# koadman/libMems

Hardware: AMD Instinct MI355X
Metric: seed-mers/sec sorted+matched (+ MUMs/sec) at 1/2/4/8 MI355X; HBM GB/s vs roofline (higher is better)
Workload: dtype u64; 1 GPU; BASELINE config 3: 8 x 100 Mbp, seed weight 19 (0x7b974ef), MemHash seed stage (sorted+matched); genomes=8, genome_length=100000000, seedmers_total=799999792, seedmers_rank0=799999792, probes_rank0=100459493, parallelism=1 GPU

## Files before the change

### libmems_amd/csrc/groups.hip

```cpp
#include <cstdlib>
#include <type_traits>

#include "match_device.h"
#include "seed_device.h"

namespace mums {

namespace {

constexpr int kGTile = kSegTile;
constexpr int kGRounds = kGTile / kBlock;
constexpr int kSlots = kGTile / 2;
#ifndef MUMS_GROUP_SPLIT
#define MUMS_GROUP_SPLIT 2
#endif
constexpr int kGSplit = MUMS_GROUP_SPLIT;
constexpr int kGSub = kGTile / kGSplit;
constexpr int kGSubRounds = kGSub / kBlock;
constexpr int kSubSlots = kGSub / 2;
static_assert(kGSub % kBlock == 0 && kGSubRounds * (kBlock / 64) <= 64, "probe sub-tile");

__device__ __forceinline__ uint32_t blk_excl_scan(uint32_t v, uint32_t* s_w, uint32_t* total) {
    const int lane = threadIdx.x & 63, wv = threadIdx.x >> 6;
    uint32_t inc = v;
// ... 88 lines not shown
    }
    if (nrep) atomicAdd(&ctr->repeat_limit, (unsigned long long)nrep);
    __syncthreads();

    uint32_t base = 0;
    const uint64_t sb = (uint64_t)blockIdx.x * kSlots;
    for (uint32_t c = 0; c < H; c += kBlock) {
        const uint32_t j = c + threadIdx.x;
        const uint32_t vv = j < H ? okb[j] : 0u;
        const uint32_t ok = vv >> 31;
        uint32_t tot;
        const uint32_t o = blk_excl_scan(ok, s_w, &tot);
        if (ok) {
            slot_info[sb + base + o] = (tile0 + heads[j]) | ((uint64_t)gsz16[j] << 32);
            slot_bucket[sb + base + o] = vv & 0x7FFFFFFFu;
        }
        base += tot;
    }
    if (threadIdx.x == 0) {
        tile_count[blockIdx.x] = base;
        tile_count[gridDim.x + 32 + blockIdx.x] = H;
    }
}

typedef __attribute__((address_space(3))) const uint64_t lds_u64;

template <int IB>
struct TileRecViewT {
    lds_u64* lds;
    const uint64_t* glob;
    uint64_t t0;
    uint32_t count;
    __device__ __forceinline__ uint64_t raw(uint64_t i) const {
        const uint64_t k = i - t0;
        return k < count ? lds[k] : glob[i];
    }
    __device__ __forceinline__ uint64_t gkey(uint64_t i) const { return raw(i) >> (IB + 1); }
    __device__ __forceinline__ uint32_t par(uint64_t i) const { return (uint32_t)(raw(i) >> IB) & 1u; }
    __device__ __forceinline__ uint64_t gidx(uint64_t i) const { return raw(i) & ((1ull << IB) - 1); }
    __device__ __forceinline__ RecFields get(uint64_t i) const {
        const uint64_t r = raw(i);
        return RecFields{r >> (IB + 1), (uint32_t)(r >> IB) & 1u, r & ((1ull << IB) - 1)};
    }
};

template <int MG, int IB, bool kGl = false, bool kFastOnly = false>
__global__ __launch_bounds__(kBlock) __attribute__((amdgpu_waves_per_eu(kGl ? 6 : 1))) void probe_tile_rec_kernel(const uint64_t* __restrict__ rec,
                                                                const SegTile* __restrict__ tiles, GenomeTable gt,
                                                                MatchParams mp, int L,
                                                                uint32_t* __restrict__ tile_count,
                                                                uint64_t* __restrict__ slot_info,
                                                                uint32_t* __restrict__ slot_bucket,
                                                                DevCounters* __restrict__ ctr,
                                                                double inv_table) {
    constexpr int kGRounds = kGSubRounds;
    constexpr int kWaves = kBlock / 64;
    __shared__ uint64_t srec[kGSub];
    __shared__ uint16_t heads[kSubSlots];
    __shared__ uint32_t wcnt[kGRounds * kWaves];
    __shared__ uint32_t s_w[2][kWaves];
    __shared__ uint32_t s_ng[kWaves];
    __shared__ uint32_t s_red[2];
    __shared__ uint64_t s_prev, s_next;
    __shared__ uint8_t s_gl[256];
    __shared__ uint32_t s_gb[kMaxG + 1];
    const int lane = threadIdx.x & 63;
    const int wv = __builtin_amdgcn_readfirstlane(threadIdx.x >> 6);
    const SegTile td = tiles[blockIdx.x / kGSplit];
    const uint32_t part0 = (blockIdx.x % kGSplit) * (uint32_t)kGSub;
    if (td.count <= part0) {
        if (threadIdx.x == 0) {
            tile_count[blockIdx.x] = 0;
            tile_count[gridDim.x + 32 + blockIdx.x] = 0;
        }
        return;
    }
    const uint64_t tile0 = td.start + part0;
    const uint32_t cnt = td.count - part0 < (uint32_t)kGSub ? td.count - part0 : (uint32_t)kGSub;

    uint32_t kx[kGRounds];
    {
        uint64_t x[kGRounds];
        #pragma unroll
        for (int r = 0; r < kGRounds; ++r) {
            const uint32_t q = r * kBlock + threadIdx.x;
            x[r] = rec[tile0 + (q < cnt ? q : cnt - 1)];
        }
        #pragma unroll
        for (int r = 0; r < kGRounds; ++r) {
            const uint32_t q = r * kBlock + threadIdx.x;
            if (q < cnt) srec[q] = x[r];
            kx[r] = (uint32_t)(x[r] >> (IB + 1));
        }
    }
    if (threadIdx.x == 0) s_prev = (tile0 > td.bstart) ? rec[tile0 - 1] : ~0ull;
    if (threadIdx.x == 64) s_next = (tile0 + cnt < td.bend) ? rec[tile0 + cnt] : ~0ull;
    constexpr bool use_gl = kGl && IB == 32;
    if constexpr (use_gl) {
        static_assert(kBlock >= 256 && kBlock > kMaxG, "one lookup entry per thread");
        if (threadIdx.x < gt.gl_n) s_gl[threadIdx.x] = gt.gl[threadIdx.x];
        if (threadIdx.x <= kMaxG) s_gb[threadIdx.x] = (uint32_t)gt.base[threadIdx.x];
    }
    const GLook glk{(lds_u8c*)s_gl, (lds_u32c*)s_gb, gt.gl_shift, gt.gl_n ? gt.gl_n - 1 : 0};
    __syncthreads();

    const bool first = tile0 == td.bstart;
    const uint32_t kprev = (uint32_t)(s_prev >> (IB + 1)), knext = (uint32_t)(s_next >> (IB + 1));
// ... 1 lines not shown
    #pragma unroll
    for (int r = 0; r < kGRounds; ++r) ke[r] = 0;
    if (lane == 0 || lane == 63) {
        #pragma unroll
        for (int r = 0; r < kGRounds; ++r) {
            const uint32_t q = r * kBlock + threadIdx.x;
            const uint32_t qe = lane == 0 ? q - 1 : q + 1;
            ke[r] = qe < cnt ? (uint32_t)(srec[qe] >> (IB + 1)) : (lane == 0 ? kprev : knext);
        }
    }
    uint32_t hmask = 0, ngrp = 0;
    #pragma unroll
    for (int r = 0; r < kGRounds; ++r) {
        const uint32_t q = r * kBlock + threadIdx.x;
        const uint32_t here = kx[r];
        const uint32_t prev = (uint32_t)__builtin_amdgcn_update_dpp((int)ke[r], (int)here, 0x138, 0xf, 0xf, false);
        uint32_t next = (uint32_t)__builtin_amdgcn_update_dpp((int)ke[r], (int)here, 0x130, 0xf, 0xf, false);
        next = (q + 1 < cnt) ? next : knext;
        const bool head = q < cnt && ((q == 0 && first) || here != prev);
        const bool keep = head && next == here;
        ngrp += (uint32_t)__popcll(__ballot(head));
        hmask |= (keep ? 1u : 0u) << r;
        const uint64_t bal = __ballot(keep);
        if (lane == 0) wcnt[r * kWaves + wv] = (uint32_t)__popcll(bal);
    }
    if (lane == 0) s_ng[wv] = ngrp;
    __syncthreads();
    if (wv == 0) {
        constexpr int kE = kGRounds * kWaves;
        const uint32_t c0 = lane < kE ? wcnt[lane] : 0u;
        uint32_t inc = c0;
        #pragma unroll
        for (int d = 1; d < 64; d <<= 1) {
            const uint32_t t = __shfl_up(inc, d, 64);
            if (lane >= d) inc += t;
        }
        if (lane < kE) wcnt[lane] = inc - c0;
        if (lane == 63) s_red[0] = inc;
    }
    __syncthreads();
    #pragma unroll
    for (int r = 0; r < kGRounds; ++r) {
        const bool keep = (hmask >> r) & 1u;
        const uint64_t bal = __ballot(keep);
        const uint32_t below = __builtin_amdgcn_mbcnt_hi((uint32_t)(bal >> 32), __builtin_amdgcn_mbcnt_lo((uint32_t)bal, 0u));
        if (keep) heads[wcnt[r * kWaves + wv] + below] = (uint16_t)(r * kBlock + threadIdx.x);
    }
    __syncthreads();
    const uint32_t H = s_red[0];

    const TileRecViewT<IB> v{(lds_u64*)srec, rec, tile0, cnt};
    const bool fast = kFastOnly || (mp.repeat_tol == 0 && mp.enum_tol == 1);
    const uint64_t want_mn = mp.masked ? mp.seq_mask : 0ull;
    const double inv_t = inv_table;
    const uint64_t sb = (uint64_t)blockIdx.x * kSubSlots;
    uint32_t nrep = 0, base = 0, buf = 0;
    for (uint32_t c = 0; c < H; c += kBlock) {
        const uint32_t j = c + threadIdx.x;
        bool ok = false;
        uint32_t gsz = 0, bkt = 0;
        uint64_t h = 0;
        if (j < H) {
            h = tile0 + heads[j];
            int64_t off = 0;
            if (fast) {
                const uint32_t q = heads[j];
                uint64_t xb[MG + 1];
                if (q + (uint32_t)gt.G < cnt) {
                    #pragma unroll
                    for (int k = 0; k <= MG; ++k) {
                        const uint32_t qk = q + ((uint32_t)k <= (uint32_t)gt.G ? (uint32_t)k : 0u);
                        xb[k] = ((uint32_t)k <= (uint32_t)gt.G) ? v.lds[qk] : ~0ull;
                    }
                } else {
                    #pragma unroll
                    for (int k = 0; k <= MG; ++k)
                        xb[k] = ((uint32_t)k <= (uint32_t)gt.G && h + k < td.bend) ? rec[h + k] : ~0ull;
                }
                ok = probe_fast_raw<MG, IB, use_gl>(xb, gt, want_mn, L, &off, &gsz, &glk);
                if (gsz > (uint32_t)gt.G) {
                    uint64_t i = h + gsz;
                    const uint32_t k0 = (uint32_t)(xb[0] >> (IB + 1));
                    while (i < td.bend && gsz <= (uint32_t)kRepeatLimit && (uint32_t)v.gkey(i) == k0) { ++gsz; ++i; }
                }
            } else if constexpr (!kFastOnly) {
                Mhe<MG> P;
                ok = build_probe<MG, TileRecViewT<IB>>(v, h, td.bend, gt, mp, L, P, &gsz);
                off = P.offset;
            }
            nrep += gsz > (uint32_t)kRepeatLimit;
            if (ok) bkt = bucket_of_fast(off, mp.table_size, inv_t);
        }
        const uint64_t bal = __ballot(ok);
        const uint32_t below = __builtin_amdgcn_mbcnt_hi((uint32_t)(bal >> 32), __builtin_amdgcn_mbcnt_lo((uint32_t)bal, 0u));
        if (lane == 0) s_w[buf][wv] = (uint32_t)__popcll(bal);
        __syncthreads();
        uint32_t pre = 0, tot = 0;
        #pragma unroll
        for (int w = 0; w < kWaves; ++w) {
            const uint32_t x = s_w[buf][w];
            pre += (w < wv) ? x : 0u;
            tot += x;
        }
        buf ^= 1u;
        if (ok) {
            const uint32_t o = base + pre + below;
            slot_info[sb + o] = h | ((uint64_t)(gsz > 65535u ? 65535u : gsz) << 32);
            slot_bucket[sb + o] = bkt;
        }
        base += tot;
    }
    if (nrep) atomicAdd(&ctr->repeat_limit, (unsigned long long)nrep);
    if (threadIdx.x == 0) {
        uint32_t gtot = 0;
        #pragma unroll
        for (int w = 0; w < kWaves; ++w) gtot += s_ng[w];
        tile_count[blockIdx.x] = base;
        tile_count[gridDim.x + 32 + blockIdx.x] = gtot;
    }
}

__global__ __launch_bounds__(kBlock) void probe_compact_kernel(const uint32_t* __restrict__ tile_count,
                                                               const uint32_t* __restrict__ tile_off,
                                                               const uint64_t* __restrict__ slot_info,
                                                               const uint32_t* __restrict__ slot_bucket,
                                                               uint64_t* __restrict__ probe_info,
                                                               uint32_t* __restrict__ probe_bucket,
                                                               uint32_t slots_per_block) {
    const uint32_t n = tile_count[blockIdx.x];
    const uint64_t o = tile_off[blockIdx.x];
    const uint64_t sb = (uint64_t)blockIdx.x * slots_per_block;
    for (uint32_t k = threadIdx.x; k < n; k += kBlock) {
        probe_info[o + k] = slot_info[sb + k];
        probe_bucket[o + k] = slot_bucket[sb + k];
    }
}

__global__ void flat_tiles_kernel(uint64_t N, uint64_t nt, SegTile* __restrict__ tiles) {
    const uint64_t t = (uint64_t)blockIdx.x * blockDim.x + threadIdx.x;
    if (t >= nt) return;
    SegTile d{};
    d.start = t * kGTile;
    d.bstart = 0;
    d.bend = N;
    const uint64_t rem = N - d.start;
    d.count = (uint32_t)(rem < (uint64_t)kGTile ? rem : (uint64_t)kGTile);
    d.hbase = 0;
    d.ntb = (uint32_t)nt;
    d.tb = (uint32_t)t;
    tiles[t] = d;
}

#ifndef MUMS_MAT_WIDE
#define MUMS_MAT_WIDE 1
#endif
constexpr bool kMatWide = MUMS_MAT_WIDE != 0;
struct __attribute__((aligned(8))) Rec2 { uint64_t a, b; };

template <int MG, typename View, bool kGl = false>
__global__ __launch_bounds__(kBlock) void probe_materialize_kernel(View v, const uint64_t* __restrict__ probe_info,
                                                                   uint64_t P, GenomeTable gt, MatchParams mp, int L,
                                                                   int64_t* __restrict__ rows, uint64_t* __restrict__ lkey,
                                                                   uint32_t* __restrict__ fsk, uint32_t* __restrict__ lhash,
                                                                   int32_t* __restrict__ rows32) {
    const uint64_t k0 = (uint64_t)blockIdx.x * kBlock;
    const uint64_t k = k0 + threadIdx.x;
    const int W = gt.G + 1;
    Mhe<MG> Q;
    __shared__ uint8_t s_gl[256];
    __shared__ uint32_t s_gb[kMaxG + 1];
    constexpr bool use_gl = kGl && RecIB<View>::value == 32;
    if constexpr (use_gl) {
        for (uint32_t i = threadIdx.x; i < gt.gl_n; i += kBlock) s_gl[i] = gt.gl[i];
        for (int i = threadIdx.x; i <= kMaxG; i += kBlock) s_gb[i] = (uint32_t)gt.base[i];
        __syncthreads();
    }
    const GLook glk{(lds_u8c*)s_gl, (lds_u32c*)s_gb, gt.gl_shift, gt.gl_n ? gt.gl_n - 1 : 0};
    if (k < P) {
        const uint64_t info = probe_info[k];
        const uint64_t h = info & 0xFFFFFFFFull;
        const uint32_t gsz = (uint32_t)((info >> 32) & 0xFFFFull);
        bool done = false;
        if constexpr (RecIB<View>::value > 0) {
            if (mp.repeat_tol == 0 && mp.enum_tol == 1 && gsz <= (uint32_t)MG) {
                uint64_t x[MG];
                if constexpr (MG % 2 == 0 && kMatWide) {
                    #pragma unroll
                    for (int q = 0; q < MG; q += 2) {
                        Rec2 t{~0ull, ~0ull};
                        if ((uint32_t)q < gsz) t = *reinterpret_cast<const Rec2*>(v.rec + h + q);
// ... 13 lines not shown
            build_probe<MG, View>(v, h, h + gsz, gt, mp, L, Q, &gs);
        }
        if (lkey) {
            const uint64_t xs = (uint64_t)start_at(Q, first_start(Q));
            if (lhash) {
                lkey[k] = (xs << 32) | k;
                lhash[k] = line_hash<MG>(Q, gt.G);
            } else {
                lkey[k] = ((uint64_t)line_hash<MG>(Q, gt.G) << 32) | (xs & 0xFFFFFFFFull);
            }
            fsk[k] = (uint32_t)xs;
        }
    }
    if constexpr (MG % 4 == 0 && MG <= 16) {
        if (rows32) {
            if (k >= P) return;
            bool ok = probe_offset<MG>(Q, L) == Q.offset;
            #pragma unroll
            for (int g = 0; g < MG; ++g) ok = ok && Q.s[g] == (int64_t)(int32_t)Q.s[g];
            int32_t* out = rows32 + k * (uint64_t)line_row_stride(gt.G);
            #pragma unroll
            for (int q = 0; q < MG / 4; ++q)
                if (4 * q < gt.G)
                    *reinterpret_cast<int4*>(out + 4 * q) = make_int4((int32_t)Q.s[4 * q], (int32_t)Q.s[4 * q + 1],
                                                                      (int32_t)Q.s[4 * q + 2], (int32_t)Q.s[4 * q + 3]);
            if (!ok) atomicOr(fsk + P, 1u);
            return;
        }
    }
    if constexpr (MG <= 16) {
        __shared__ int64_t srow[kBlock * (MG + 1)];
        if (k < P) {
            int64_t* r = srow + threadIdx.x * W;
            #pragma unroll
            for (int g = 0; g < MG; ++g)
                if (g < gt.G) r[g] = Q.s[g];
            r[gt.G] = Q.offset;
        }
        __syncthreads();
        const uint64_t nk = P - k0 < (uint64_t)kBlock ? P - k0 : (uint64_t)kBlock;
        int64_t* out = rows + k0 * (uint64_t)W;
        for (uint32_t i = threadIdx.x; i < nk * (uint64_t)W; i += kBlock) out[i] = srow[i];
    } else {
        if (k >= P) return;
        int64_t* row = rows + k * (uint64_t)W;
        #pragma unroll
        for (int g = 0; g < MG; ++g)
            if (g < gt.G) row[g] = Q.s[g];
        row[gt.G] = Q.offset;
    }
}

__global__ __launch_bounds__(kBlock) void row_bucket_kernel(const int64_t* __restrict__ rows, uint64_t P, int G,
                                                            uint32_t table_size, double inv_t,
                                                            const uint32_t* __restrict__ bounds, uint32_t nranks,
                                                            uint32_t* __restrict__ out) {
    const uint64_t k = (uint64_t)blockIdx.x * kBlock + threadIdx.x;
    if (k >= P) return;
    const uint32_t b = bucket_of_fast(rows[k * (uint64_t)(G + 1) + G], table_size, inv_t);
    if (!bounds) { out[k] = b; return; }
    uint32_t r = 0;
    while (r + 1 < nranks && bounds[r + 1] <= b) ++r;
    out[k] = r;
}

constexpr int kGatherIPT = 8;
__global__ __launch_bounds__(kBlock) void gather_rows_ilp_kernel(const int64_t* __restrict__ src,
                                                                 const uint32_t* __restrict__ perm, uint64_t n, uint32_t W,
                                                                 int64_t* __restrict__ dst) {
    const uint64_t e0 = (uint64_t)blockIdx.x * (kBlock * kGatherIPT) + threadIdx.x;
    uint64_t k = e0 / W;
    uint32_t c = (uint32_t)(e0 - k * W);
    const uint32_t dk = kBlock / W, dc = kBlock % W;
    int64_t x[kGatherIPT];
    #pragma unroll
    for (int i = 0; i < kGatherIPT; ++i) {
        const uint64_t e = e0 + (uint64_t)i * kBlock;
        x[i] = e < n ? src[(uint64_t)perm[k] * W + c] : 0;
        k += dk;
        c += dc;
        if (c >= W) { c -= W; ++k; }
    }
    #pragma unroll
    for (int i = 0; i < kGatherIPT; ++i) {
        const uint64_t e = e0 + (uint64_t)i * kBlock;
        if (e < n) dst[e] = x[i];
    }
}

__global__ __launch_bounds__(kBlock) void bucket_rec_kernel(const uint32_t* __restrict__ b, uint64_t P,
                                                            uint64_t* __restrict__ rec) {
    const uint64_t k = (uint64_t)blockIdx.x * kBlock + threadIdx.x;
    if (k < P) rec[k] = ((uint64_t)b[k] << 32) | k;
}

__global__ __launch_bounds__(kBlock) void bucket_split_kernel(const uint64_t* __restrict__ rec, uint64_t P,
                                                              uint32_t* __restrict__ b, uint32_t* __restrict__ ids) {
    const uint64_t k = (uint64_t)blockIdx.x * kBlock + threadIdx.x;
    if (k >= P) return;
    const uint64_t r = rec[k];
    b[k] = (uint32_t)(r >> 32);
    ids[k] = (uint32_t)r;
}

__global__ __launch_bounds__(kBlock) void chain_dest_kernel(const uint32_t* __restrict__ fk, uint64_t nch,
                                                            const uint32_t* __restrict__ pdest,
                                                            uint32_t* __restrict__ cdest) {
    const uint64_t c = (uint64_t)blockIdx.x * kBlock + threadIdx.x;
    if (c < nch) cdest[c] = pdest[fk[c]];
}

__global__ __launch_bounds__(kBlock) void inverse_perm_kernel(const uint32_t* __restrict__ perm, uint64_t n,
                                                              uint32_t* __restrict__ inv) {
    const uint64_t k = (uint64_t)blockIdx.x * kBlock + threadIdx.x;
    if (k < n) inv[perm[k]] = (uint32_t)k;
}

__global__ __launch_bounds__(kBlock) void chain_tag_kernel(const uint32_t* __restrict__ chain_of,
                                                           const uint32_t* __restrict__ perm,
                                                           const uint32_t* __restrict__ sdest, uint64_t P,
                                                           const uint32_t* __restrict__ cinv,
                                                           const uint32_t* __restrict__ cstart,
                                                           uint32_t* __restrict__ tags) {
    const uint64_t k = (uint64_t)blockIdx.x * kBlock + threadIdx.x;
    if (k < P) tags[k] = cinv[chain_of[perm[k]]] - cstart[sdest[k]];
}

__global__ __launch_bounds__(kBlock) void chain_entry_out_kernel(const int64_t* __restrict__ pool,
                                                                 const uint32_t* __restrict__ fk,
                                                                 const uint32_t* __restrict__ cperm,
                                                                 const uint32_t* __restrict__ scdest, uint64_t nch,
                                                                 int G, const uint32_t* __restrict__ pinv,
                                                                 const uint32_t* __restrict__ rstart,
                                                                 int64_t* __restrict__ eout, uint32_t* __restrict__ fout) {
    const uint64_t k = (uint64_t)blockIdx.x * kBlock + threadIdx.x;
    if (k >= nch) return;
    const uint32_t c = cperm[k];
    const uint64_t W = (uint64_t)(G + 2);
    for (uint64_t w = 0; w < W; ++w) eout[k * W + w] = pool[(uint64_t)c * W + w];
    if (fout) fout[k] = pinv[fk[c]] - rstart[scdest[k]];
}

__global__ __launch_bounds__(kBlock) void kept_dest_kernel(const int64_t* __restrict__ rows, uint64_t P, int G,
                                                           const uint32_t* __restrict__ chain_of,
                                                           const uint32_t* __restrict__ cinv,
                                                           const uint2* __restrict__ thr,
                                                           const uint32_t* __restrict__ fk,
                                                           const uint32_t* __restrict__ pdest, uint32_t nranks,
                                                           uint32_t* __restrict__ dest) {
    const uint64_t k = (uint64_t)blockIdx.x * kBlock + threadIdx.x;
    if (k >= P) return;
    const uint32_t c = chain_of[k];
    const uint2 t = thr[cinv[c]];
    bool keep = t.y != 0u && fk[c] == (uint32_t)k;
    if (!keep) {
// ... 73 lines not shown

hipError_t launch_inverse_perm(const uint32_t* perm, uint64_t n, uint32_t* inv, hipStream_t st) {
    if (n == 0) return hipSuccess;
    hipLaunchKernelGGL(inverse_perm_kernel, dim3((unsigned)((n + kBlock - 1) / kBlock)), dim3(kBlock), 0, st, perm, n,
                       inv);
    return hipGetLastError();
}

hipError_t launch_chain_tags(const uint32_t* chain_of, const uint32_t* perm, const uint32_t* sdest, uint64_t P,
                             const uint32_t* cinv, const uint32_t* cstart, uint32_t* tags, hipStream_t st) {
    if (P == 0) return hipSuccess;
    hipLaunchKernelGGL(chain_tag_kernel, dim3((unsigned)((P + kBlock - 1) / kBlock)), dim3(kBlock), 0, st, chain_of,
                       perm, sdest, P, cinv, cstart, tags);
    return hipGetLastError();
}

hipError_t launch_chain_entries_out(const int64_t* pool, const uint32_t* fk, const uint32_t* cperm,
                                    const uint32_t* scdest, uint64_t nch, int G, const uint32_t* pinv,
                                    const uint32_t* rstart, int64_t* eout, uint32_t* fout, hipStream_t st) {
    if (nch == 0) return hipSuccess;
    hipLaunchKernelGGL(chain_entry_out_kernel, dim3((unsigned)((nch + kBlock - 1) / kBlock)), dim3(kBlock), 0, st,
                       pool, fk, cperm, scdest, nch, G, pinv, rstart, eout, fout);
    return hipGetLastError();
}

hipError_t launch_kept_dest(const int64_t* rows, uint64_t P, int G, const uint32_t* chain_of, const uint32_t* cinv,
                            const uint2* thr, const uint32_t* fk, const uint32_t* pdest, uint32_t nranks, uint32_t* dest,
                            hipStream_t st) {
    if (P == 0) return hipSuccess;
    hipLaunchKernelGGL(kept_dest_kernel, dim3((unsigned)((P + kBlock - 1) / kBlock)), dim3(kBlock), 0, st, rows, P, G,
                       chain_of, cinv, thr, fk, pdest, nranks, dest);
    return hipGetLastError();
}

hipError_t launch_dest_first(const uint32_t* sdest, uint64_t P, uint32_t* first, hipStream_t st) {
    if (P == 0) return hipSuccess;
    hipLaunchKernelGGL(dest_first_kernel, dim3((unsigned)((P + kBlock - 1) / kBlock)), dim3(kBlock), 0, st, sdest, P,
                       first);
    return hipGetLastError();
}

hipError_t launch_entry_first(const uint32_t* scdest, uint64_t nch, const uint32_t* rcount, const uint32_t* perm,
                              const uint32_t* sdest, uint64_t K, const uint32_t* chain_of, const uint32_t* cinv,
                              const uint32_t* rstart, uint32_t* efirst, hipStream_t st) {
    if (nch == 0) return hipSuccess;
    hipLaunchKernelGGL(entry_first_init_kernel, dim3((unsigned)((nch + kBlock - 1) / kBlock)), dim3(kBlock), 0, st,
                       scdest, nch, rcount, efirst);
    if (K)
        hipLaunchKernelGGL(entry_first_kernel, dim3((unsigned)((K + kBlock - 1) / kBlock)), dim3(kBlock), 0, st, perm,
                           sdest, K, chain_of, cinv, rstart, efirst);
    return hipGetLastError();
}

hipError_t launch_bucket_records(const uint32_t* b, uint64_t P, uint64_t* rec, hipStream_t st) {
    if (P == 0) return hipSuccess;
    hipLaunchKernelGGL(bucket_rec_kernel, dim3((unsigned)((P + kBlock - 1) / kBlock)), dim3(kBlock), 0, st, b, P, rec);
    return hipGetLastError();
}

hipError_t launch_bucket_split(const uint64_t* rec, uint64_t P, uint32_t* b, uint32_t* ids, hipStream_t st) {
    if (P == 0) return hipSuccess;
    hipLaunchKernelGGL(bucket_split_kernel, dim3((unsigned)((P + kBlock - 1) / kBlock)), dim3(kBlock), 0, st, rec, P, b,
                       ids);
    return hipGetLastError();
}

uint64_t group_slot_count(uint64_t ntiles) { return ntiles * kSlots; }
uint64_t group_blocks(uint64_t ntiles, bool packed) { return packed ? ntiles * kGSplit : ntiles; }

template <int MG, typename View>
hipError_t launch_materialize(View v, const uint64_t* probe_info, uint64_t P, const GenomeTable& gt,
                              const MatchParams& mp, int L, int64_t* rows, hipStream_t st, uint64_t* lkey,
                              uint32_t* fsk, uint32_t* lhash, int32_t* rows32) {
    if (P == 0) return hipSuccess;
    if (RecIB<View>::value == 32 && gt.gl_n > 0)
        hipLaunchKernelGGL((probe_materialize_kernel<MG, View, true>), dim3((unsigned)((P + kBlock - 1) / kBlock)),
                           dim3(kBlock), 0, st, v, probe_info, P, gt, mp, L, rows, lkey, fsk, lhash, rows32);
    else
        hipLaunchKernelGGL((probe_materialize_kernel<MG, View>), dim3((unsigned)((P + kBlock - 1) / kBlock)),
                           dim3(kBlock), 0, st, v, probe_info, P, gt, mp, L, rows, lkey, fsk, lhash, rows32);
    return hipGetLastError();
}

hipError_t launch_row_buckets(const int64_t* rows, uint64_t P, int G, uint32_t table_size, const uint32_t* d_bounds,
                              uint32_t nranks, uint32_t* out, hipStream_t st) {
    if (P == 0) return hipSuccess;
    hipLaunchKernelGGL(row_bucket_kernel, dim3((unsigned)((P + kBlock - 1) / kBlock)), dim3(kBlock), 0, st, rows, P, G,
                       table_size, 1.0 / (double)table_size, d_bounds, nranks, out);
    return hipGetLastError();
}

hipError_t launch_gather_rows(const int64_t* src, const uint32_t* perm, uint64_t P, int G, int64_t* dst,
                              hipStream_t st) {
    if (P == 0) return hipSuccess;
    const uint64_t n = P * (uint64_t)(G + 1);
    const uint64_t per = (uint64_t)kBlock * kGatherIPT;
    hipLaunchKernelGGL(gather_rows_ilp_kernel, dim3((unsigned)((n + per - 1) / per)), dim3(kBlock), 0, st, src, perm, n,
                       (uint32_t)(G + 1), dst);
    return hipGetLastError();
}

hipError_t launch_flat_tiles(uint64_t N, SegTile* d_tiles, hipStream_t st) {
    const uint64_t nt = (N + kGTile - 1) / kGTile;
    if (nt == 0) return hipSuccess;
    hipLaunchKernelGGL(flat_tiles_kernel, dim3((unsigned)((nt + 255) / 256)), dim3(256), 0, st, N, nt, d_tiles);
    return hipGetLastError();
}

template <int MG, typename View>
hipError_t launch_probe_tiles(View v, const SegTile* tiles, uint64_t ntiles, uint64_t N, const GenomeTable& gt,
                              const MatchParams& mp, int L, uint32_t* tile_count, uint64_t* slot_info,
                              uint32_t* slot_bucket, void* counters, hipStream_t st) {
    if (ntiles == 0) return hipSuccess;
    if constexpr (RecIB<View>::value > 0) {
        const bool fast = mp.repeat_tol == 0 && mp.enum_tol == 1;
        const double inv_t = 1.0 / (double)mp.table_size;
        if (RecIB<View>::value == 32 && gt.gl_n > 0 && fast && !getenv("MUMS_DEV_PROBE_GENERAL"))
            hipLaunchKernelGGL((probe_tile_rec_kernel<MG, RecIB<View>::value, true, true>),
                               dim3((unsigned)(ntiles * kGSplit)), dim3(kBlock), 0, st, v.rec, tiles, gt, mp, L,
                               tile_count, slot_info, slot_bucket, (DevCounters*)counters, inv_t);
        else if (RecIB<View>::value == 32 && gt.gl_n > 0)
            hipLaunchKernelGGL((probe_tile_rec_kernel<MG, RecIB<View>::value, true>), dim3((unsigned)(ntiles * kGSplit)),
                               dim3(kBlock), 0, st, v.rec, tiles, gt, mp, L, tile_count, slot_info, slot_bucket,
                               (DevCounters*)counters, inv_t);
        else
            hipLaunchKernelGGL((probe_tile_rec_kernel<MG, RecIB<View>::value>), dim3((unsigned)(ntiles * kGSplit)),
                               dim3(kBlock), 0, st, v.rec, tiles, gt, mp, L, tile_count, slot_info, slot_bucket,
                               (DevCounters*)counters, inv_t);
    } else
        hipLaunchKernelGGL((probe_tile_kernel<MG, View>), dim3((unsigned)ntiles), dim3(kBlock), 0, st, v, tiles, N, gt,
                           mp, L, tile_count, slot_info, slot_bucket, (DevCounters*)counters);
    return hipGetLastError();
}

hipError_t launch_probe_compact(uint64_t nblocks, const uint32_t* tile_count, const uint32_t* tile_off,
                                const uint64_t* slot_info, const uint32_t* slot_bucket, uint64_t* probe_info,
                                uint32_t* probe_bucket, hipStream_t st, bool packed) {
    if (nblocks == 0) return hipSuccess;
    hipLaunchKernelGGL(probe_compact_kernel, dim3((unsigned)nblocks), dim3(kBlock), 0, st, tile_count, tile_off,
                       slot_info, slot_bucket, probe_info, probe_bucket, (uint32_t)(packed ? kSubSlots : kSlots));
    return hipGetLastError();
}

#define MUMS_INST_PROBE(MG, V)                                                                                     \
    template hipError_t launch_probe_tiles<MG, V>(V, const SegTile*, uint64_t, uint64_t, const GenomeTable&,      \
                                                  const MatchParams&, int, uint32_t*, uint64_t*, uint32_t*, void*, \
                                                  hipStream_t);
MUMS_INST_PROBE(4, PairView<uint32_t>)
MUMS_INST_PROBE(8, PairView<uint32_t>)
MUMS_INST_PROBE(16, PairView<uint32_t>)
MUMS_INST_PROBE(32, PairView<uint32_t>)
MUMS_INST_PROBE(64, PairView<uint32_t>)
MUMS_INST_PROBE(4, PairView<uint64_t>)
MUMS_INST_PROBE(8, PairView<uint64_t>)
MUMS_INST_PROBE(16, PairView<uint64_t>)
MUMS_INST_PROBE(32, PairView<uint64_t>)
MUMS_INST_PROBE(64, PairView<uint64_t>)
#define MUMS_INST_MAT(MG, V)                                                                                      \
    template hipError_t launch_materialize<MG, V>(V, const uint64_t*, uint64_t, const GenomeTable&,                \
                                                  const MatchParams&, int, int64_t*, hipStream_t, uint64_t*,      \
                                                  uint32_t*, uint32_t*, int32_t*);
MUMS_INST_MAT(4, PairView<uint32_t>)
MUMS_INST_MAT(8, PairView<uint32_t>)
MUMS_INST_MAT(16, PairView<uint32_t>)
MUMS_INST_MAT(32, PairView<uint32_t>)
MUMS_INST_MAT(64, PairView<uint32_t>)
MUMS_INST_MAT(4, PairView<uint64_t>)
MUMS_INST_MAT(8, PairView<uint64_t>)
MUMS_INST_MAT(16, PairView<uint64_t>)
MUMS_INST_MAT(32, PairView<uint64_t>)
MUMS_INST_MAT(64, PairView<uint64_t>)
MUMS_INST_MAT(4, RecView)
MUMS_INST_MAT(8, RecView)
MUMS_INST_MAT(16, RecView)
MUMS_INST_MAT(32, RecView)
MUMS_INST_MAT(64, RecView)
MUMS_INST_PROBE(4, RecView)
MUMS_INST_PROBE(8, RecView)
MUMS_INST_PROBE(16, RecView)
MUMS_INST_PROBE(32, RecView)
MUMS_INST_PROBE(64, RecView)
MUMS_INST_MAT(4, RecViewT<33>)
MUMS_INST_MAT(8, RecViewT<33>)
MUMS_INST_MAT(16, RecViewT<33>)
MUMS_INST_MAT(32, RecViewT<33>)
MUMS_INST_MAT(64, RecViewT<33>)
MUMS_INST_PROBE(4, RecViewT<33>)
MUMS_INST_PROBE(8, RecViewT<33>)
MUMS_INST_PROBE(16, RecViewT<33>)
MUMS_INST_PROBE(32, RecViewT<33>)
MUMS_INST_PROBE(64, RecViewT<33>)
// ... 3 lines not shown
```

### libmems_amd/csrc/match_device.h

```cpp
#pragma once

#include <type_traits>

#include "mums_internal.h"
#include "seed_device.h"

namespace mums {

template <int MG>
struct Mhe {
    int64_t len;
    int64_t offset;
    int64_t mersize;
    int64_t s[MG];
};

template <int MG>
__device__ __forceinline__ int first_start(const Mhe<MG>& m) {
    int f = MG;
    #pragma unroll
    for (int g = MG - 1; g >= 0; --g) f = (m.s[g] != 0) ? g : f;
    return f;
}

template <int MG>
__device__ __forceinline__ int64_t start_at(const Mhe<MG>& m, int i) {
    int64_t v = 0;
    #pragma unroll
    for (int g = 0; g < MG; ++g) v = (g == i) ? m.s[g] : v;
    return v;
}

template <int MG>
__device__ __forceinline__ bool mhe_contains(const Mhe<MG>& a, const Mhe<MG>& b) {
    if (a.offset != b.offset) return false;
    const int i = first_start(b);
    const int64_t ai = start_at(a, i), bi = start_at(b, i);
    if (ai == 0) return false;
    const int64_t diff = bi - ai;
    if (diff < 0 || (uint64_t)a.len < (uint64_t)(b.len + diff)) return false;
    const int64_t diff_rc = b.len - a.len + diff;
    bool ok = true;
    #pragma unroll
    for (int g = 0; g < MG; ++g) {
        if (g <= i) continue;
        const int64_t di = b.s[g] - a.s[g];
        if (b.s[g] == 0 && a.s[g] == 0) continue;
        if (b.s[g] < 0 && diff_rc == di) continue;
        if (diff != di) ok = false;
    }
    return ok;
}

template <int MG>
// ... 157 lines not shown
        while (i < end && cnt <= (uint32_t)kRepeatLimit && v.gkey(i) == k0) { ++cnt; ++i; }
        *gsize = cnt;
        return false;
    }
    *gsize = cnt;
    if (cnt < 2) return false;
    MaskT<MG> mask = 0;
    bool dup = false;
    int gref = 64;
    int64_t sref = 0;
    uint32_t pref = 0;
    int gk[MG + 1];
    #pragma unroll
    for (int k = 0; k <= MG; ++k) {
        gk[k] = genome_of_mg<MG>(gt, r[k].idx);
        if ((uint32_t)k < cnt) {
            const int g = gk[k];
            dup = dup || ((mask >> g) & 1u);
            mask |= (MaskT<MG>)1 << g;
            if (g < gref) {
                gref = g;
                sref = (int64_t)(r[k].idx - gt.base[g]) + 1;
                pref = r[k].par;
            }
        }
    }
    if (dup) return false;
    int64_t off = 0;
    #pragma unroll
    for (int k = 0; k <= MG; ++k) {
        if ((uint32_t)k < cnt && gk[k] != gref) {
            const int64_t s = (int64_t)(r[k].idx - gt.base[gk[k]]) + 1;
            off += (r[k].par != pref) ? (-s - sref - (int64_t)L) : (s - sref);
        }
    }
    *offset = off;
    if (mp.masked) {
        const uint64_t match_number = match_number_of(mask, G);
        return mp.seq_mask == 0 || match_number == mp.seq_mask;
    }
    return true;
}

template <int MG, typename View>
__device__ __forceinline__ bool probe_offset_fast(const View& v, uint64_t h, uint64_t end, const GenomeTable& gt,
                                                  const MatchParams& mp, int L, int64_t* offset, uint32_t* gsize) {
    RecFields r[MG + 1];
    #pragma unroll
    for (int k = 0; k <= MG; ++k)
        r[k] = ((uint32_t)k <= (uint32_t)gt.G && h + k < end) ? v.get(h + k) : RecFields{~0ull, 0u, 0u};
    return probe_offset_batch<MG, View>(r, v, h, end, gt, mp, L, offset, gsize);
}

__device__ __forceinline__ uint32_t bucket_of_fast(int64_t offset, uint32_t table_size, double inv_t) {
    const int64_t T = (int64_t)table_size;
    const int64_t q = (int64_t)floor((double)offset * inv_t);
    int64_t r = offset - q * T;
    r = r < 0 ? r + T : r;
    r = r >= T ? r - T : r;
    return (uint32_t)r;
}

typedef __attribute__((address_space(3))) const uint8_t lds_u8c;
typedef __attribute__((address_space(3))) const uint32_t lds_u32c;
struct GLook {
    lds_u8c* tab;
    lds_u32c* base;
    uint32_t shift, last;
};
__device__ __forceinline__ void glook(const GLook& l, uint32_t idx, uint32_t* g, uint32_t* b) {
    const uint32_t s = min(idx >> l.shift, l.last);
    const uint32_t t = l.tab[s];
    const uint32_t b0 = l.base[t], b1 = l.base[t + 1];
    const bool ge = idx >= b1;
    *g = t + (ge ? 1u : 0u);
    *b = ge ? b1 : b0;
}

template <int MG, int IB, bool kGl, typename IdxT>
__device__ __forceinline__ void rec_genome_start(uint64_t x, const GenomeTable& gt, const GLook* glk, uint32_t* g_out,
                                                 IdxT* s_out) {
    const IdxT idx = (IdxT)(x & ((1ull << IB) - 1));
    uint32_t g = 0;
    IdxT b = 0;
    if constexpr (kGl && IB == 32) {
        uint32_t bb;
        glook(*glk, (uint32_t)idx, &g, &bb);
        b = bb;
    } else {
        const uint32_t G = (uint32_t)gt.G;
        #pragma unroll
        for (int j = 1; j < MG; ++j) {
            const IdxT bj = (IdxT)gt.base[j];
            const bool ge = (uint32_t)j < G && idx >= bj;
            g = ge ? (uint32_t)j : g;
            b = ge ? bj : b;
        }
    }
    *g_out = g;
    *s_out = idx - b + 1u;
}

template <int MG, int IB = 32, bool kGl = false>
__device__ __forceinline__ bool probe_fast_raw(const uint64_t (&x)[MG + 1], const GenomeTable& gt, uint64_t want_mn,
                                               int L, int64_t* offset, uint32_t* gsize,
                                               const GLook* glk = nullptr) {
    const uint32_t G = (uint32_t)gt.G;
    const uint32_t k0 = (uint32_t)(x[0] >> (IB + 1));
    uint32_t cnt = 0;
    bool run = true;
    #pragma unroll
    for (int k = 0; k <= MG; ++k) {
        run = run && ((uint32_t)(x[k] >> (IB + 1)) == k0) && (x[k] != ~0ull);
        cnt += run ? 1u : 0u;
// ... 192 lines not shown
```

### libmems_amd/csrc/mums_capi.hip

```cpp
#include <hip/hip_runtime.h>

#include <algorithm>
#include <array>
#include <chrono>
#include <functional>
#include <cstddef>
#include <cstdio>
#include <cstdlib>
#include <cstring>
#include <memory>
#include <string>
#include <vector>

#include "../../include/mums.h"
#include "match_device.h"
#include "mums_internal.h"
#include "seed_device.h"

using namespace mums;

namespace {

struct DevBuf {
    void* p = nullptr;
// ... 36 lines not shown

struct GenomeIn {
    const char* d_ptr;
    uint64_t n;
    bool owned;
};

enum { EV_START, EV_KEYS, EV_SORT, EV_GROUPS, EV_BUCKETS, EV_CHAINS, EV_REPLAY, EV_OUTPUT, EV_COUNT };

constexpr uint32_t kReplayLdsIds = 8192;

}

struct mums_ctx {
    int device = 0;
    hipStream_t stream = nullptr;
    bool own_stream = false;
    uint64_t seed = 0;
    uint32_t repeat_tol = 0, enum_tol = 1, table_size = 40000;
    int masked = 0;
    uint64_t seq_mask = 0;
    std::vector<GenomeIn> genomes;
    std::string err;

    DevBuf packed, recA, recB, hist, tiles, ckey, kA, kB, vA, vB, tmp, partials, counters;
    DevBuf bstart, bend, tsize, obase, pool, tbl, out_len, out_s, pbuf, keybuf, mstart;
    DevBuf cmerge;
    DevBuf chain_tmp, chain_of, radix_tmp, spill, summ, dbgbuf, mprobe, rowtmp;
    DevBuf fk, fkloc;
    DevBuf side, bst8;
    DevBuf cbst;
    bool use_onesweep = true;
    bool pcompat = false;
    bool compat_rec = false;
    uint32_t compat_rank = 0, compat_ranks = 1;
    mums_ctx* compat_sub = nullptr;
    DevBuf rkpool0, rkpool1, rku32, ascii_all;
    bool prelabelled = false;
    uint64_t prelab_n = 0;
    const int64_t* lab_rows = nullptr;
    uint64_t lab_nch = 0;
    uint64_t lab_p = 0;
    double lab_ms = 0;
    uint32_t kx_nranks = 0;
    std::vector<uint32_t> kx_estart;
    uint64_t own_rows = 0;
    uint64_t own_dropped = 0;
    bool kept_rows = false;
    bool pairwise = false;
    uint64_t chunk_size = 200000;
    uint32_t nchunks = 0;
    DevBuf cval, ctab;
    DevBuf fsk;
    DevBuf bst2;
    bool fused_keys = false;
    bool rows_narrow = false;
    DevBuf smlk0, smlkA, smlkB, smlvA, smlvB, smltmp, flen, fs;
    DevBuf rowsall;
    DevBuf pool_loc, cbuf;
    DevBuf sids;
    DevBuf labx;
    uint32_t* emit_tbl = nullptr;
    const uint32_t* emit_base = nullptr;
    EoWork eo;
    bool match_log = false;
    uint64_t log_n = 0;
    DevBuf logA, logB, logvA, logvB;
    std::vector<uint64_t> start_points;
    DevBuf rsbuf, rsplan, rsbst;
    DevBuf tiebuf;
    DevBuf crbuf, crcnt, crlive, crruns;
    uint64_t cr_cands = 0;
    DevBuf crall;
    bool shard_restart_pending = false;
    uint64_t live_n = 0;
    std::vector<uint32_t> live_bst;
    int shard_mb = 0;
    int shard_side = 0;
    uint64_t shard_n = 0;
    uint32_t shard_kfirst = 0, shard_kcount = 0;
    std::vector<uint32_t> shard_bst;
    DevBuf dsarr;
    bool ds_ready = false;
    uint64_t ds_C = 0;
    std::vector<uint64_t> ds_n, ds_off;
    std::vector<uint64_t> ds_rkey, ds_rS;
    bool ds_ties = false;
    uint64_t rs_info[4] = {0, 0, 0, 0};
    bool ties_fixed = false;
    uint64_t tie_slots = 0;
    int keep_tiebuf = 0;
    bool tiebuf_kept = false;
    uint64_t restarts = 0;
    std::vector<uint64_t> offset_log;
    std::vector<uint64_t> consumed_log;
    std::vector<uint32_t> compat_pfirst;
    std::vector<uint32_t> log_ids;
    bool log_host = false;
    std::vector<uint64_t> log_hlen;
    std::vector<int64_t> log_hs;
    std::vector<uint64_t> compat_cons;
    const uint64_t* compat_ck_src = nullptr;
    uint64_t compat_ck_mask = 0;
    bool progress_on = false;
    std::string progress;
    hipEvent_t ev[EV_COUNT] = {};
    bool profiling = false;
// ... 47 lines not shown
}

int hipfail(mums_ctx* c, hipError_t e, const char* where) {
    return fail(c, e == hipErrorOutOfMemory ? MUMS_E_NOMEM : MUMS_E_HIP,
                std::string(where) + ": " + hipGetErrorString(e));
}

#define HIPCHK(expr)                                               \
    do {                                                           \
        hipError_t e_ = (expr);                                    \
        if (e_ != hipSuccess) return hipfail(ctx, e_, #expr);      \
    } while (0)

bool have_device() {
    int n = 0;
    return hipGetDeviceCount(&n) == hipSuccess && n > 0;
}

SeedSpec make_seed_spec(uint64_t pattern, int L, int w) {
    SeedSpec ss{};
    ss.pattern = pattern;
    ss.L = L;
    ss.w = w;
    int cum = 0, r = -1;
    bool prev = false;
    for (int k = 0; k < L; ++k) {
        const bool care = (pattern >> (L - 1 - k)) & 1;
        if (care) {
            if (!prev) {
                ++r;
                ss.run_start[r] = k;
                ss.run_len[r] = 0;
            }
            ss.run_len[r]++;
        }
        prev = care;
    }
    ss.nruns = r + 1;
    for (int i = 0; i < ss.nruns; ++i) {
        cum += ss.run_len[i];
        ss.run_dst[i] = 2 * (w - cum);
        ss.run_sh[i] = 64 - 2 * (ss.run_start[i] + ss.run_len[i]) - ss.run_dst[i];
        ss.run_mask[i] = ((ss.run_len[i] >= 32) ? ~0ull : ((1ull << (2 * ss.run_len[i])) - 1)) << ss.run_dst[i];
    }
    return ss;
}

int seed_len(uint64_t s) {
    if (!s) return 0;
    int lo = __builtin_ctzll(s), hi = 63 - __builtin_clzll(s);
    return hi - lo + 1;
}

template <int MG, typename View>
int run_groups(mums_ctx* ctx, View v, const SegTile* tiles, uint64_t ntiles, const MatchParams& mp,
               uint64_t* probe_info, uint32_t* probe_bucket, uint64_t* slot_info, uint32_t* slot_bucket,
               hipStream_t st) {
    const bool packed = RecIB<View>::value > 0;
    const uint64_t nb = group_blocks(ntiles, packed);
    uint32_t* counts = ctx->partials.as<uint32_t>();
    uint32_t* gcounts = counts + nb + 32;
    uint32_t* offs = gcounts + nb + 32;
    DevCounters* dc = ctx->counters.as<DevCounters>();
    HIPCHK((launch_probe_tiles<MG, View>(v, tiles, ntiles, ctx->N, ctx->gt, mp, ctx->L, counts, slot_info, slot_bucket,
                                         dc, st)));
    HIPCHK(exclusive_scan_u32(gcounts, nb, ctx->tmp.p, &dc->ngroups, st));
    HIPCHK(hipMemcpyAsync(offs, counts, nb * 4, hipMemcpyDeviceToDevice, st));
    HIPCHK(exclusive_scan_u32(offs, nb, ctx->tmp.p, &dc->nprobes, st));
    HIPCHK(launch_probe_compact(nb, counts, offs, slot_info, slot_bucket, probe_info, probe_bucket, st, packed));
    return MUMS_OK;
}

template <typename View>
int groups_dispatch(mums_ctx* ctx, View v, const SegTile* tiles, uint64_t ntiles, const MatchParams& mp,
                    uint64_t* pi, uint32_t* pb, uint64_t* si, uint32_t* sb, hipStream_t st) {
    const int G = ctx->gt.G;
    if (G <= 4) return run_groups<4, View>(ctx, v, tiles, ntiles, mp, pi, pb, si, sb, st);
    if (G <= 8) return run_groups<8, View>(ctx, v, tiles, ntiles, mp, pi, pb, si, sb, st);
    if (G <= 16) return run_groups<16, View>(ctx, v, tiles, ntiles, mp, pi, pb, si, sb, st);
    if (G <= 32) return run_groups<32, View>(ctx, v, tiles, ntiles, mp, pi, pb, si, sb, st);
    return run_groups<64, View>(ctx, v, tiles, ntiles, mp, pi, pb, si, sb, st);
}

void* devbuf_alloc(void* b, size_t bytes) {
    DevBuf* d = (DevBuf*)b;
    return d->ensure(bytes) == hipSuccess ? d->p : nullptr;
}

template <int MG>
int find_replay(mums_ctx* ctx, MatProbes v, const MatchParams& mp, hipStream_t st);

template <int MG>
int find_rows(mums_ctx* ctx, MatProbes v, const uint32_t* packed, const MatchParams& mp, hipStream_t st) {
    DevCounters* dc = ctx->counters.as<DevCounters>();
    const uint64_t P = ctx->P;
    HIPCHK(ctx->fk.ensure((P + 1) * 4));
    HIPCHK((launch_chains<MG, MatProbes>(v, nullptr, P, ctx->gt, mp, ctx->ss, packed,
                                    ctx->chain_tmp.p, ctx->tmp.p, ctx->radix_tmp.p, nullptr,
                                    ctx->pool.as<int64_t>(), &dc->nchains, st, dc,
                                    ctx->profiling ? ctx->ev_walk : nullptr, ctx->fk.as<uint32_t>(), 0u,
                                    v.fs != nullptr, ctx->chain_of.as<uint32_t>())));
    return find_replay<MG>(ctx, v, mp, st);
}

template <int MG>
int find_replay(mums_ctx* ctx, MatProbes v, const MatchParams& mp, hipStream_t st) {
    DevCounters* dc = ctx->counters.as<DevCounters>();
    const uint64_t P = ctx->P;
    ctx->walk_events = ctx->profiling;
    HIPCHK(hipEventRecord(ctx->ev[EV_CHAINS], st));
    HIPCHK(hipMemcpyAsync(&ctx->hc, dc, sizeof(DevCounters), hipMemcpyDeviceToHost, st));
    HIPCHK(hipStreamSynchronize(st));
    uint64_t* dbg = nullptr;
    if (getenv("MUMS_DEV_REPLAY_DEBUG")) {
        HIPCHK(ctx->dbgbuf.ensure((size_t)ctx->table_size * 64));
        HIPCHK(hipMemsetAsync(ctx->dbgbuf.p, 0, (size_t)ctx->table_size * 64, st));
        dbg = ctx->dbgbuf.as<uint64_t>();
    }
    uint64_t* mlog = nullptr;
    ctx->log_n = 0;
    if (ctx->match_log) {
        HIPCHK(ctx->logA.ensure((P + 1) * 8));
        HIPCHK(ctx->logB.ensure((P + 1) * 8));
        mlog = ctx->logB.as<uint64_t>();
    }
    const uint32_t lds_cap = std::max<uint32_t>(64, std::min<uint32_t>(ctx->hc.max_bucket, kReplayLdsIds));
    HIPCHK((launch_replay_kept<MG, MatProbes>(v, ctx->gt, mp, ctx->L, P, ctx->pool.as<int64_t>(), nullptr,
                                         ctx->fk.as<uint32_t>(), ctx->hc.nchains,
                                         ctx->chain_tmp.p, ctx->radix_tmp.p, ctx->tmp.p, lds_cap,
                                         ctx->tsize.as<uint32_t>(), ctx->counters.p, dbg, st, mlog, &ctx->emit_tbl,
                                         &ctx->emit_base, devbuf_alloc, &ctx->cbuf, ctx->chain_of.as<uint32_t>())));
    if (mlog) {
        HIPCHK(hipMemcpyAsync(&ctx->hc, dc, sizeof(DevCounters), hipMemcpyDeviceToHost, st));
        HIPCHK(hipStreamSynchronize(st));
// ... 320 lines not shown
                HIPCHK(ctx->chain_tmp.ensure(cbytes));
            for (DevBuf* b : {&ctx->pbuf, &ctx->tiles, &ctx->rowtmp, &ctx->kA, &ctx->kB, &ctx->vA, &ctx->vB,
                              &ctx->ckey, &ctx->mprobe})
                if (!(b->p && (char*)v.rows >= (char*)b->p && (char*)v.rows < (char*)b->p + b->cap)) b->release();
            if (!arena) {
                ctx->recA.release();
                ctx->recB.release();
            }
        }
        rc = find_rows_dispatch(ctx, v, packed, mp, st, chunked);
        if (rc) return rc;
        if (ctx->pcompat) {
            HIPCHK(hipMemcpyAsync(ctx->obase.p, ctx->tsize.p, (size_t)Tb * 4, hipMemcpyDeviceToDevice, st));
            HIPCHK(exclusive_scan_u32(ctx->obase.as<uint32_t>(), Tb, ctx->tmp.p, &dc->nmatches, st));
            uint32_t tot = 0;
            HIPCHK(hipMemcpyAsync(&tot, &dc->nmatches, 4, hipMemcpyDeviceToHost, st));
            HIPCHK(hipStreamSynchronize(st));
            HIPCHK(ctx->cmerge.ensure((size_t)Tb * 4 + 64));
            HIPCHK(launch_compat_merge(ctx->tsize.as<uint32_t>(), ctx->emit_base, ctx->emit_tbl,
                                       ctx->pool.as<int64_t>(), G, Tb, &dc->collisions, ctx->obase.as<uint32_t>(), tot,
                                       ctx->cmerge.as<uint32_t>(), st));
        }
    }
    HIPCHK(hipEventRecord(ctx->ev[EV_REPLAY], st));
    HIPCHK(hipMemcpyAsync(ctx->obase.p, ctx->tsize.p, (size_t)Tb * 4, hipMemcpyDeviceToDevice, st));
    HIPCHK(exclusive_scan_u32(ctx->obase.as<uint32_t>(), Tb, ctx->tmp.p, &dc->nmatches, st));
    HIPCHK(hipMemcpyAsync(&ctx->hc, dc, sizeof(DevCounters), hipMemcpyDeviceToHost, st));
    HIPCHK(hipStreamSynchronize(st));
    if (ctx->hc.err & 4u) return fail(ctx, MUMS_E_HIP, "bucket replay: an insert broke the rank order (internal error)");
    ctx->M = ctx->hc.nmatches;
    HIPCHK(ctx->out_len.ensure((ctx->M + 1) * 8));
    HIPCHK(ctx->out_s.ensure((ctx->M + 1) * (size_t)G * 8));
    HIPCHK(launch_emit(ctx->obase.as<uint32_t>(), ctx->emit_base, ctx->emit_tbl,
                       ctx->pool.as<int64_t>(), G, Tb, ctx->M, ctx->out_len.as<uint64_t>(), ctx->out_s.as<int64_t>(),
                       st));
    HIPCHK(hipEventRecord(ctx->ev[EV_OUTPUT], st));
    ctx->log_ids.clear();
    if (ctx->match_log && ctx->pcompat) {
        const int rc = compat_log_order(ctx, Tb, st);
        if (rc) return rc;
    }
    ctx->stage_done = MUMS_STAGE_ALL;
    return MUMS_OK;
}

struct ProbeSpace {
    uint64_t* probe_info;
    uint64_t* slot_info;
    uint32_t* probe_bucket;
    uint32_t* bucketB;
    uint32_t* idsA;
    uint32_t* idsB;
    uint32_t* slot_bucket;
};

int ensure_probe_space(mums_ctx* ctx, uint64_t N, uint64_t ntiles_groups, ProbeSpace* ps) {
    const uint64_t pcap = (N / 2 + 2) & ~1ull;
    const uint64_t nslots = group_slot_count(ntiles_groups);
    HIPCHK(ctx->partials.ensure((3 * group_blocks(ntiles_groups, true) + 128) * 4));
    HIPCHK(ctx->pbuf.ensure(pcap * (8 + 4 * 4) + nslots * 12 + 256));
    char* pb = (char*)ctx->pbuf.p;
    ps->probe_info = (uint64_t*)pb;
    ps->slot_info = ps->probe_info + pcap;
    ps->probe_bucket = (uint32_t*)(ps->slot_info + nslots);
    ps->bucketB = ps->probe_bucket + pcap;
    ps->idsA = ps->bucketB + pcap;
    ps->idsB = ps->idsA + pcap;
    ps->slot_bucket = ps->idsB + pcap;
    return MUMS_OK;
}

uint32_t layout_packed(GenomeTable& t, uint64_t* words) {
    uint64_t wsum = 0;
    uint32_t T = 0;
    for (int g = 0; g < t.G; ++g) {
        t.woff[g] = wsum;
        wsum += (packed_words(t.n[g]) + 3) & ~3ull;
        t.tfirst[g] = T;
        T += (uint32_t)((t.n[g] + kSeedTile - 1) / kSeedTile);
    }
    t.woff[t.G] = wsum;
    for (int g = t.G; g <= kMaxG; ++g) t.tfirst[g] = T;
    *words = wsum;
    return T;
}

int keys_stage(mums_ctx* ctx, const GenomeTable& lgt, uint32_t T, int B, uint64_t n, uint64_t* out, uint32_t* bstart,
               hipStream_t st, int ib = 32, int side = 0) {
    DevCounters* dc = ctx->counters.as<DevCounters>();
    std::vector<const char*> ptrs(lgt.G);
    for (int g = 0; g < lgt.G; ++g) ptrs[g] = ctx->genomes[g].d_ptr;
    uint32_t* hist = ctx->hist.as<uint32_t>();
    if (side > 0) {
        if (B != 8 + side || out == ctx->recB.as<uint64_t>() || (ib != 32 && ib != 33))
            return fail(ctx, MUMS_E_INVALID, "msd split");
        HIPCHK(ctx->side.ensure(n + 64));
        HIPCHK(ctx->bst8.ensure((256 + 64) * 4));
        HIPCHK(ctx->recB.ensure(n * 8 + 64));
        HIPCHK(ctx->tmp.ensure(std::max(ctx->tmp.cap, msd_split_tmp_bytes(n, 8))));
        HIPCHK(launch_seed_pack(ctx->ss, lgt, ptrs.data(), ctx->packed.as<uint32_t>(), 1, true, nullptr, 8, hist, T,
                                &dc->err, st));
        HIPCHK(exclusive_scan_u32(hist, (uint64_t)T << 8, ctx->tmp.p, nullptr, st));
        if (ib == 32) {
            HIPCHK(launch_seed_scatter(ctx->ss, lgt, ctx->packed.as<uint32_t>(), 8, hist, T, ctx->recB.as<uint64_t>(),
                                       st, ctx->side.as<uint8_t>(), side));
        } else {
            HIPCHK(ctx->ctab.ensure(64));
            HIPCHK(hipMemsetAsync(ctx->ctab.p, 0, 64, st));
            HIPCHK(launch_seed_scatter_chunk(ctx->ss, lgt, ctx->packed.as<uint32_t>(), 8, hist, T, 0, 0,
                                             ctx->recB.as<uint64_t>(), st, ctx->ctab.as<uint64_t>(), 8,
                                             ctx->side.as<uint8_t>(), side));
        }
        HIPCHK(seg_bucket_starts(hist, T, 8, n, ctx->bst8.as<uint32_t>(), st));
        HIPCHK(msd_split(ctx->recB.as<uint64_t>(), ctx->side.as<uint8_t>(), out, n, 8, side, ctx->bst8.as<uint32_t>(),
                         bstart, ctx->tmp.p, st));
        return MUMS_OK;
    }
    HIPCHK(launch_seed_pack(ctx->ss, lgt, ptrs.data(), ctx->packed.as<uint32_t>(), 1, true, nullptr, B, hist, T,
                            &dc->err, st));
    if (B > 0) HIPCHK(exclusive_scan_u32(hist, (uint64_t)T << B, ctx->tmp.p, nullptr, st));
    if (ib == 32) {
        HIPCHK(launch_seed_scatter(ctx->ss, lgt, ctx->packed.as<uint32_t>(), B, hist, T, out, st));
    } else {
        HIPCHK(ctx->ctab.ensure(64));
        HIPCHK(hipMemsetAsync(ctx->ctab.p, 0, 64, st));
        HIPCHK(launch_seed_scatter_chunk(ctx->ss, lgt, ctx->packed.as<uint32_t>(), B, hist, T, 0, 0, out, st,
                                         ctx->ctab.as<uint64_t>(), B));
    }
    HIPCHK(seg_bucket_starts(B > 0 ? hist : nullptr, T, B, n, bstart, st));
    return MUMS_OK;
}

void records_live(mums_ctx* ctx) {
    for (DevBuf* b : {&ctx->rowtmp, &ctx->sids, &ctx->summ, &ctx->chain_tmp}) b->drop_view();
}

int ensure_merge_space(mums_ctx* ctx, uint64_t n, int mb, int key_bits, ProbeSpace* ps) {
    records_live(ctx);
    const uint64_t ub = seg_tiles_upper(n, mb);
    HIPCHK(ctx->recA.ensure(n * 8 + 64));
    HIPCHK(ctx->recB.ensure(n * 8 + 64));
    HIPCHK(ctx->tiles.ensure(ub * sizeof(SegTile) + 64));
    HIPCHK(ctx->mstart.ensure(((1ull << mb) + 64) * 4));
    size_t tmpb = std::max(seg_tmp_bytes(n, mb), onesweep_tmp_bytes(n, mb, key_bits));
    tmpb = std::max(tmpb, std::max(scan_tmp_bytes(n), radix_tmp_bytes(n / 2 + 1)));
    tmpb = std::max(tmpb, scan_tmp_bytes((uint64_t)ctx->table_size));
    HIPCHK(ctx->tmp.ensure(tmpb));
    return ensure_probe_space(ctx, n, ub, ps);
}

int tie_fix_stream(mums_ctx* ctx, const RsStream& s, uint64_t n, hipStream_t st);
bool wants_tie_order(const mums_ctx* ctx);

int merge_stage(mums_ctx* ctx, uint64_t n, int mb, int key_bits, const MatchParams& mp, const ProbeSpace& ps,
                hipStream_t st, int ib = 32, uint64_t* rA = nullptr, uint64_t* rB = nullptr) {
    DevCounters* dc = ctx->counters.as<DevCounters>();
    if (!rA) rA = ctx->recA.as<uint64_t>();
    if (!rB) rB = ctx->recB.as<uint64_t>();
    SegTile* tiles = ctx->tiles.as<SegTile>();
    const uint32_t* bstart = ctx->mstart.as<uint32_t>();
    const uint64_t ub = seg_tiles_upper(n, mb);
    const bool prof = ctx->profiling;
    HIPCHK(build_seg_tiles_from_starts(bstart, mb, n, tiles, &dc->ntiles, ctx->tmp.p, st));
    int buf = 0;
    if (ib != 32 && !(n < (1ull << 30) && key_bits <= 32))
        return fail(ctx, MUMS_E_UNSUPPORTED, "33-bit records need < 2^30 records per merge");
    const bool mask_parity = mp.repeat_tol == 0 && mp.enum_tol == 1;
    ctx->parity_masked = false;
    const bool onesweep = ctx->use_onesweep && n < (1ull << 30) && key_bits <= 32;
    const bool wide = onesweep && mask_parity && ib == 32 && seg_wide_sort_enabled() && seg_wide_passes(key_bits) <= 3;
    if (wide) {
        HIPCHK(seg_onesweep_sort_wide(rA, rB, n, key_bits, mb, bstart, ctx->tmp.p, &dc->err, &buf, st,
                                      prof ? ctx->ev_ds : nullptr, 32));
        ctx->parity_masked = true;
    } else if (onesweep) {
        HIPCHK(seg_onesweep_sort(rA, rB, n, key_bits, mb, bstart, ctx->tmp.p, &dc->err, &buf, st,
                                 prof ? ctx->ev_ds : nullptr, ib, mask_parity));
        ctx->parity_masked = mask_parity && seg_onesweep_launches(key_bits) < (key_bits + 7) / 8;
    } else
        HIPCHK(seg_radix_sort(rA, rB, n, key_bits, tiles, ub, ctx->tmp.p, &buf, st, prof ? ctx->ev_ds : nullptr));
    ctx->sorted_buf = buf;
    ctx->sorted_rec = buf ? rB : rA;
    ctx->sort_passes = wide ? seg_wide_passes(key_bits) : onesweep ? seg_onesweep_launches(key_bits) : (key_bits + 7) / 8;
    HIPCHK(hipEventRecord(ctx->ev[EV_SORT], st));
    if (wants_tie_order(ctx) && ib == 32 && !ctx->shard) {
        RsStream s{};
        s.kind = 0;
        s.rec = ctx->sorted_rec;
        s.bstart = bstart;
        s.B = mb;
        s.kbits = 2 * ctx->w + 1;
        const int rc = tie_fix_stream(ctx, s, n, st);
        if (rc) return rc;
    }
    if (ib == 33)
        return groups_dispatch<RecViewT<33>>(ctx, RecViewT<33>{ctx->sorted_rec}, tiles, ub, mp, ps.probe_info,
                                             ps.probe_bucket, ps.slot_info, ps.slot_bucket, st);
    return groups_dispatch<RecView>(ctx, RecView{ctx->sorted_rec}, tiles, ub, mp, ps.probe_info, ps.probe_bucket,
                                    ps.slot_info, ps.slot_bucket, st);
}

int finish_seeds(mums_ctx* ctx, const ProbeSpace& ps, hipStream_t st, bool find_follows = false) {
    DevCounters* dc = ctx->counters.as<DevCounters>();
    HIPCHK(hipMemcpyAsync(&ctx->hc, dc, sizeof(DevCounters), hipMemcpyDeviceToHost, st));
    HIPCHK(hipStreamSynchronize(st));
    if (ctx->hc.err & 1u) return fail(ctx, MUMS_E_GAP, "Gap in genome sequence ('-' encountered)");
    if (ctx->hc.err & 2u) return fail(ctx, MUMS_E_HIP, "sort look-back timed out (internal error)");
    if (ctx->hc.err & 16u) return fail(ctx, MUMS_E_HIP, "sort segment fix-up list overflow (internal error)");
    ctx->P = ctx->hc.nprobes;
    ctx->probe_info = ps.probe_info;
    HIPCHK(hipEventRecord(ctx->ev[EV_GROUPS], st));
    int tbits = 1;
    while (tbits < 32 && ((uint64_t)1 << tbits) < (uint64_t)ctx->table_size) ++tbits;
    const uint64_t P = ctx->P;
    if (find_follows && P > 0 && P <= find_chunk() && !ctx->shard && !getenv("MUMS_DEV_KEEP_BUCKET_ORDER")) {
        ctx->sorted_buckets = nullptr;
        ctx->sorted_ids = nullptr;
        HIPCHK(hipEventRecord(ctx->ev[EV_BUCKETS], st));
        return MUMS_OK;
    }
    const bool radix = getenv("MUMS_DEV_BUCKET_ONESWEEP") == nullptr;
    if (!radix && P >= 4096 && P < (1ull << 30) && ps.slot_info + P <= (const uint64_t*)ps.probe_bucket &&
        ctx->tmp.cap >= onesweep_tmp_bytes(P, 0, tbits)) {
        uint64_t* rA = ps.slot_info;
        uint64_t* rB = (uint64_t*)ps.bucketB;
        HIPCHK(ctx->bst2.ensure(64));
        HIPCHK(launch_bucket_records(ps.probe_bucket, P, rA, st));
        HIPCHK(seg_bucket_starts(nullptr, 0, 0, P, ctx->bst2.as<uint32_t>(), st));
        int ob = 0;
        HIPCHK(seg_onesweep_sort(rA, rB, P, tbits, 0, ctx->bst2.as<uint32_t>(), ctx->tmp.p, &dc->err, &ob, st));
        HIPCHK(launch_bucket_split(ob ? rB : rA, P, ps.probe_bucket, ps.idsB, st));
        ctx->sorted_buckets = ps.probe_bucket;
        ctx->sorted_ids = ps.idsB;
    } else {
        int pout = 0;
        HIPCHK(radix_sort<uint32_t>(ps.probe_bucket, nullptr, P, tbits, ps.bucketB, ps.idsA, ps.probe_bucket,
                                    ps.idsB, ctx->tmp.p, &pout, st));
        ctx->sorted_buckets = pout ? ps.probe_bucket : ps.bucketB;
        ctx->sorted_ids = pout ? ps.idsB : ps.idsA;
    }
    HIPCHK(hipEventRecord(ctx->ev[EV_BUCKETS], st));
    return MUMS_OK;
}

void fill_stats(mums_ctx* ctx, uint64_t n) {
    struct ClearLast {
        ~ClearLast() { (void)hipGetLastError(); }
    } clear_last;
    mums_stats& s = ctx->st;
    s = mums_stats{};
    s.seedmers = n;
    s.groups = ctx->hc.ngroups;
    s.probes = ctx->P;
    s.repeat_limit_groups = ctx->hc.repeat_limit;
    s.restarts = ctx->restarts;
    auto el = [&](int a, int b) {
        float ms = 0.f;
        (void)hipEventElapsedTime(&ms, ctx->ev[a], ctx->ev[b]);
        return (double)ms;
    };
    const size_t kb = ctx->key64 ? 8 : 4;
    const int passes = ctx->sort_passes;
    s.ms_keys = el(EV_START, EV_KEYS);
    s.ms_sort = el(EV_KEYS, EV_SORT);
    s.ms_groups = el(EV_SORT, EV_GROUPS);
    s.ms_buckets = el(EV_GROUPS, EV_BUCKETS);
    s.key_bytes = ctx->packed_path ? 8 : kb;
    s.sort_passes = (uint64_t)passes;
    if (ctx->profiling && n > 0) {
        for (int p = 0; p < passes; ++p) {
            float ms = 0.f;
            (void)hipEventElapsedTime(&ms, ctx->ev_ds[2 * p], ctx->ev_ds[2 * p + 1]);
            s.ms_dominant += ms;
            s.dominant_bytes += ctx->packed_path ? n * 16 : n * (kb + (p ? 4 : 0) + kb + 4);
        }
        s.dominant_launches = (uint64_t)passes;
    }
    s.chunks = ctx->nchunks;
    if (ctx->stage_done >= MUMS_STAGE_ALL) {
        s.mem_count = ctx->pcompat ? ctx->M : ctx->hc.entries;
        s.collision_count = ctx->hc.collisions;
        s.ms_chains = el(EV_BUCKETS, EV_CHAINS);
        s.ms_replay = el(EV_CHAINS, EV_REPLAY);
        s.chains = ctx->hc.nchains;
        s.ms_output = el(EV_REPLAY, EV_OUTPUT);
        s.ms_total = el(EV_START, EV_OUTPUT);
// ... 234 lines not shown
    hipStream_t st = ctx->stream;
    const int G = (int)ctx->genomes.size();
    const uint64_t N = ctx->N;
    MatchParams mp{ctx->repeat_tol, ctx->enum_tol, ctx->table_size, ctx->masked, ctx->seq_mask};
    GenomeTable& gt = ctx->gt;

    uint64_t words = 0;
    const uint32_t T = layout_packed(gt, &words);
    HIPCHK(ctx->packed.ensure(words * 4 + 64));
    HIPCHK(ctx->counters.ensure(sizeof(DevCounters)));
    DevCounters* dc = ctx->counters.as<DevCounters>();
    const SeedSpec& ss = ctx->ss;

    const int kbits = 2 * ctx->w + 1;
    ctx->packed_path = kbits <= 32 + kMaxMsdBits;
    ctx->msd_bits = ctx->packed_path ? std::max(0, kbits - 32) : 0;
    if (const char* e = getenv("MUMS_DEV_MSD_BITS"))
        if (ctx->packed_path) ctx->msd_bits = std::min(kMaxMsdBits, std::max(ctx->msd_bits, atoi(e)));
    if (ctx->packed_path && seg_wide_sort_enabled() && ctx->msd_bits < 8 && kbits - 8 <= 31 && kbits > 8 &&
        ctx->repeat_tol == 0 && ctx->enum_tol == 1)
        ctx->msd_bits = 8;
    const int B = ctx->msd_bits;
    const int side = (ctx->packed_path && B > 8 && !getenv("MUMS_DEV_MSD_BITS") && !getenv("MUMS_DEV_NO_SPLIT"))
                         ? B - 8 : 0;
    const size_t kb = ctx->key64 ? 8 : 4;
    ProbeSpace ps{};
    if (ctx->packed_path) {
        HIPCHK(ctx->hist.ensure(((uint64_t)T << B) * 4 + 64));
        HIPCHK(ctx->tmp.ensure(scan_tmp_bytes((uint64_t)T << B)));
        int rc0 = ensure_merge_space(ctx, N, B, kbits - B, &ps);
        if (rc0) return rc0;
        HIPCHK(ctx->tmp.ensure(std::max(scan_tmp_bytes((uint64_t)T << B), ctx->tmp.cap)));
    } else {
        const uint64_t ntiles_groups = (N + kSegTile - 1) / kSegTile;
        HIPCHK(ctx->ckey.ensure(N * kb + 64));
        HIPCHK(ctx->kA.ensure(N * kb + 64));
        HIPCHK(ctx->kB.ensure(N * kb + 64));
        HIPCHK(ctx->vA.ensure(N * 4 + 64));
        HIPCHK(ctx->vB.ensure(N * 4 + 64));
        HIPCHK(ctx->tiles.ensure(ntiles_groups * sizeof(SegTile) + 64));
        size_t tmpb = std::max(scan_tmp_bytes(N), radix_tmp_bytes(N));
        tmpb = std::max(tmpb, scan_tmp_bytes((uint64_t)ctx->table_size));
        HIPCHK(ctx->tmp.ensure(tmpb));
        int rc0 = ensure_probe_space(ctx, N, ntiles_groups, &ps);
        if (rc0) return rc0;
    }

    HIPCHK(hipEventRecord(ctx->ev[EV_START], st));
    HIPCHK(hipMemsetAsync(dc, 0, sizeof(DevCounters), st));
    const bool prof = ctx->profiling;
    if (prof && !ctx->ev_ds[0])
        for (int i = 0; i < 16; ++i) HIPCHK(hipEventCreate(&ctx->ev_ds[i]));

    int rc = MUMS_OK;
    if (ctx->packed_path) {
        rc = keys_stage(ctx, gt, T, B, N, ctx->recA.as<uint64_t>(), ctx->mstart.as<uint32_t>(), st, 32, side);
        if (rc) return rc;
        HIPCHK(hipEventRecord(ctx->ev[EV_KEYS], st));
        rc = merge_stage(ctx, N, B, kbits - B, mp, ps, st);
    } else {
        std::vector<const char*> ptrs(G);
        for (int g = 0; g < G; ++g) ptrs[g] = ctx->genomes[g].d_ptr;
        HIPCHK(launch_seed_pack(ss, gt, ptrs.data(), ctx->packed.as<uint32_t>(), 0, ctx->key64, ctx->ckey.p, 0,
                                nullptr, T, &dc->err, st));
        HIPCHK(hipEventRecord(ctx->ev[EV_KEYS], st));
        int buf = 0;
        SegTile* tiles = ctx->tiles.as<SegTile>();
        const uint64_t ntiles_groups = (N + kSegTile - 1) / kSegTile;
        HIPCHK(launch_flat_tiles(N, tiles, st));
        if (ctx->key64) {
            HIPCHK(radix_sort<uint64_t>(ctx->ckey.as<uint64_t>(), nullptr, N, kbits, ctx->kA.as<uint64_t>(),
                                        ctx->vA.as<uint32_t>(), ctx->kB.as<uint64_t>(), ctx->vB.as<uint32_t>(),
                                        ctx->tmp.p, &buf, st, prof ? ctx->ev_ds : nullptr));
        } else {
            HIPCHK(radix_sort<uint32_t>(ctx->ckey.as<uint32_t>(), nullptr, N, kbits, ctx->kA.as<uint32_t>(),
                                        ctx->vA.as<uint32_t>(), ctx->kB.as<uint32_t>(), ctx->vB.as<uint32_t>(),
                                        ctx->tmp.p, &buf, st, prof ? ctx->ev_ds : nullptr));
        }
        ctx->sorted_buf = buf;
        ctx->sorted_key = buf ? ctx->kB.p : ctx->kA.p;
        ctx->sorted_idx = buf ? ctx->vB.as<uint32_t>() : ctx->vA.as<uint32_t>();
        ctx->sort_passes = (kbits + 7) / 8;
        HIPCHK(hipEventRecord(ctx->ev[EV_SORT], st));
        if (wants_tie_order(ctx)) {
            RsStream s{};
            s.kind = ctx->key64 ? 2 : 1;
            s.key = ctx->sorted_key;
            s.idx = ctx->sorted_idx;
            rc = tie_fix_stream(ctx, s, N, st);
            if (rc) return rc;
        }
        if (ctx->key64)
            rc = groups_dispatch<PairView<uint64_t>>(ctx, PairView<uint64_t>{(const uint64_t*)ctx->sorted_key,
                                                                             ctx->sorted_idx},
                                                     tiles, ntiles_groups, mp, ps.probe_info, ps.probe_bucket,
                                                     ps.slot_info, ps.slot_bucket, st);
        else
            rc = groups_dispatch<PairView<uint32_t>>(ctx, PairView<uint32_t>{(const uint32_t*)ctx->sorted_key,
                                                                             ctx->sorted_idx},
                                                     tiles, ntiles_groups, mp, ps.probe_info, ps.probe_bucket,
                                                     ps.slot_info, ps.slot_bucket, st);
    }
    if (rc) return rc;
    rc = finish_seeds(ctx, ps, st, stage >= MUMS_STAGE_ALL);
    if (rc) return rc;
    rc = restart_stage(ctx, mp, ps, st);
    if (rc) return rc;
    ctx->stage_done = MUMS_STAGE_SEEDS;

    if (stage >= MUMS_STAGE_ALL) {
        rc = find_tail(ctx, mp, ctx->packed.as<uint32_t>(), [&](MatProbes* v) {
            const int r = materialize_seeds(ctx, mp, st);
            v->rows = ctx->mprobe.as<int64_t>();
            return r;
        }, st, true);
        if (rc) return rc;
    }
    HIPCHK(hipStreamSynchronize(st));
    HIPCHK(hipMemcpy(&ctx->hc, dc, sizeof(DevCounters), hipMemcpyDeviceToHost));

    fill_stats(ctx, N);
    return MUMS_OK;
}

int prepare_run(mums_ctx* ctx, const std::vector<uint64_t>& lens) {
    records_live(ctx);
    ctx->stage_done = 0;
    ctx->compat_rec = false;
    ctx->ties_fixed = false;
    ctx->tie_slots = 0;
    ctx->restarts = 0;
    ctx->offset_log.clear();
    ctx->log_host = false;
    ctx->M = ctx->P = 0;
    const int G = (int)lens.size();
    uint64_t total = 0;
    for (uint64_t n : lens) total += n;
    uint64_t pat = ctx->seed;
    if (pat == 0) {
        uint32_t wdef = mums_default_seed_weight(G ? total / (uint64_t)G : 0);
        pat = (uint64_t)mums_get_seed((int)wdef, 0);
    }
    const int L = seed_len(pat), w = __builtin_popcountll(pat);
    if (L == 0) return fail(ctx, MUMS_E_INVALID, "Can't have 0 seed length");
    if (L > 32) return fail(ctx, MUMS_E_INVALID, "Mer size is too large");
    if (w > 31) return fail(ctx, MUMS_E_UNSUPPORTED, "seed weight 32 not supported");
    ctx->pattern = pat;
    ctx->L = L;
    ctx->w = w;
    ctx->key64 = (2 * w + 1) > 32;
    GenomeTable& gt = ctx->gt;
    gt = GenomeTable{};
    gt.G = G;
    uint64_t N = 0;
    for (int g = 0; g < G; ++g) {
        gt.n[g] = lens[g];
        gt.m[g] = gt.n[g] < (uint64_t)L ? 0 : gt.n[g] - L + 1;
// ... 555 lines not shown
        }
        for (int g = (int)nl; g <= kMaxG; ++g) l.base[g] = ctx->gt.base[ctx->shard_first + nl];
    }
    ctx->packed_path = true;
    ctx->msd_bits = shard_msd_bits(ctx->w);
    const bool big = ctx->gt.base[ctx->gt.G] >= 0xFFFFFFF0ull || getenv("MUMS_DEV_SHARD_IB33") != nullptr;
    ctx->rec_ib = big ? 33 : 32;
    ctx->shard_side = 0;
    if (big && 2 * ctx->w + 1 - 31 > 8 && 2 * ctx->w + 1 - 31 <= 12) {
        ctx->msd_bits = 2 * ctx->w + 1 - 31;
        ctx->shard_side = ctx->msd_bits - 8;
    } else if (big && (2 * ctx->w + 1 - ctx->msd_bits != 31 || ctx->msd_bits > 8)) {
        return fail(ctx, MUMS_E_UNSUPPORTED, "sharded mode above 2^32 seed-mers needs seed weight 19-21");
    }
    return MUMS_OK;
}

}

extern "C" {

int mums_abi_version(void) { return MUMS_ABI_VERSION; }

int mums_ctx_create(int device, mums_ctx** out) {
    if (!out) return MUMS_E_INVALID;
    *out = nullptr;
    if (!have_device()) return MUMS_E_NODEVICE;
    mums_ctx* ctx = new mums_ctx();
    ctx->device = device;
    hipError_t e = hipSetDevice(device);
    if (e != hipSuccess) { delete ctx; return MUMS_E_HIP; }
    e = hipStreamCreateWithFlags(&ctx->stream, hipStreamNonBlocking);
    if (e != hipSuccess) { delete ctx; return MUMS_E_HIP; }
    ctx->own_stream = true;
    for (int i = 0; i < EV_COUNT; ++i) (void)hipEventCreate(&ctx->ev[i]);
    for (int i = 0; i < 6; ++i) (void)hipEventCreate(&ctx->ev_walk[i]);
    *out = ctx;
    return MUMS_OK;
}

int mums_ctx_destroy(mums_ctx* ctx) {
    if (!ctx) return MUMS_E_INVALID;
    (void)hipSetDevice(ctx->device);
    mums_clear(ctx);
    DevBuf* bufs[] = {&ctx->packed, &ctx->recA, &ctx->recB, &ctx->hist, &ctx->tiles, &ctx->ckey, &ctx->kA,
                      &ctx->kB, &ctx->vA, &ctx->vB, &ctx->tmp, &ctx->partials, &ctx->counters, &ctx->bstart,
                      &ctx->bend, &ctx->tsize, &ctx->obase, &ctx->pool, &ctx->tbl, &ctx->out_len, &ctx->out_s,
                      &ctx->pbuf, &ctx->keybuf, &ctx->mstart, &ctx->chain_tmp, &ctx->chain_of,
                      &ctx->radix_tmp, &ctx->spill, &ctx->summ, &ctx->dbgbuf, &ctx->mprobe, &ctx->rowtmp,
                      &ctx->cval, &ctx->ctab, &ctx->smlk0, &ctx->smlkA, &ctx->smlkB, &ctx->smlvA,
                      &ctx->smlvB, &ctx->smltmp, &ctx->flen, &ctx->fs, &ctx->rowsall, &ctx->rsbuf,
                      &ctx->rsplan, &ctx->rsbst, &ctx->pool_loc, &ctx->cbuf, &ctx->sids,
                      &ctx->logA, &ctx->logB, &ctx->logvA, &ctx->logvB, &ctx->tiebuf, &ctx->fk, &ctx->fkloc,
                      &ctx->crbuf, &ctx->crcnt, &ctx->crlive, &ctx->crruns, &ctx->crall, &ctx->fsk, &ctx->bst2,
                      &ctx->side, &ctx->bst8, &ctx->cbst, &ctx->dsarr, &ctx->labx, &ctx->rkpool0, &ctx->rkpool1,
                      &ctx->rku32, &ctx->ascii_all};
    for (DevBuf* b : bufs) b->release();
    for (int i = 0; i < EV_COUNT; ++i)
        if (ctx->ev[i]) (void)hipEventDestroy(ctx->ev[i]);
    for (int i = 0; i < 16; ++i)
        if (ctx->ev_ds[i]) (void)hipEventDestroy(ctx->ev_ds[i]);
    for (int i = 0; i < 6; ++i)
        if (ctx->ev_walk[i]) (void)hipEventDestroy(ctx->ev_walk[i]);
    if (ctx->compat_sub) (void)mums_ctx_destroy(ctx->compat_sub);
    if (ctx->own_stream && ctx->stream) (void)hipStreamDestroy(ctx->stream);
    delete ctx;
    return MUMS_OK;
}

int mums_set_stream(mums_ctx* ctx, void* s) {
    if (check_ctx(ctx)) return MUMS_E_INVALID;
    if (!s) return fail(ctx, MUMS_E_INVALID, "null stream");
    if (ctx->own_stream && ctx->stream) (void)hipStreamDestroy(ctx->stream);
    ctx->stream = (hipStream_t)s;
    ctx->own_stream = false;
    return MUMS_OK;
}

int mums_set_seed(mums_ctx* ctx, uint64_t pattern) {
    if (check_ctx(ctx)) return MUMS_E_INVALID;
    ctx->seed = pattern;
    return MUMS_OK;
}

int mums_set_params(mums_ctx* ctx, uint32_t repeat_tol, uint32_t enum_tol, uint32_t table_size) {
    if (check_ctx(ctx)) return MUMS_E_INVALID;
    if (table_size == 0 || table_size > 0x7FFFFFFFu)
        return fail(ctx, MUMS_E_INVALID, "table size must be in [1, 2^31)");
    ctx->repeat_tol = repeat_tol;
    ctx->enum_tol = enum_tol;
    ctx->table_size = table_size;
    return MUMS_OK;
}

int mums_set_mask(mums_ctx* ctx, int masked, uint64_t seq_mask) {
    if (check_ctx(ctx)) return MUMS_E_INVALID;
    ctx->masked = masked ? 1 : 0;
    ctx->seq_mask = seq_mask;
    return MUMS_OK;
}

int mums_add_genome(mums_ctx* ctx, const char* ascii, uint64_t n) {
    if (check_ctx(ctx)) return MUMS_E_INVALID;
    if (!ascii && n) return fail(ctx, MUMS_E_INVALID, "Null gnSequence pointer");
    if (ctx->genomes.size() >= (size_t)kMaxG)
        return fail(ctx, MUMS_E_UNSUPPORTED, "more than 64 genomes per context");
    HIPCHK(hipSetDevice(ctx->device));
// ... 1761 lines not shown
    if (check_ctx(ctx) || !vofs || (ctx->shard_n && !d_ids)) return MUMS_E_INVALID;
    if (!ctx->ds_ready) return fail(ctx, MUMS_E_INVALID, "mums_shard_restart_prepare first");
    HIPCHK(hipSetDevice(ctx->device));
    hipStream_t st = ctx->stream;
    const uint64_t W = (uint64_t)ctx->gt.G + 1;
    uint64_t* d_vofs = ctx->dsarr.as<uint64_t>() + 9 * W;
    HIPCHK(hipMemcpyAsync(d_vofs, vofs, (W - 1) * 8, hipMemcpyHostToDevice, st));
    CrStream s{ctx->sorted_rec, ctx->crbuf.as<uint64_t>(), 1u << ctx->msd_bits, ctx->shard_n};
    s.kb = (uint32_t)(2 * ctx->w + 1 - ctx->msd_bits);
    s.ib = (uint32_t)ctx->rec_ib;
    HIPCHK(launch_cr_tie_vals(s, ctx->gt, ctx->crcnt.as<uint32_t>(), d_vofs, d_ids,
                              const_cast<uint64_t*>(ctx->sorted_rec), st));
    HIPCHK(hipStreamSynchronize(st));
    ctx->ds_ties = true;
    ctx->ties_fixed = true;
    return MUMS_OK;
}

int mums_shard_restart_info(mums_ctx* ctx, uint64_t* info) {
    if (check_ctx(ctx) || !info) return MUMS_E_INVALID;
    std::copy(ctx->rs_info, ctx->rs_info + 4, info);
    return MUMS_OK;
}

int mums_probe_count(mums_ctx* ctx, uint64_t* count) {
    if (check_ctx(ctx) || !count) return MUMS_E_INVALID;
    if (ctx->stage_done < MUMS_STAGE_SEEDS) return fail(ctx, MUMS_E_INVALID, "no seed stage run");
    if (ctx->shard && ctx->shard_restart_pending)
        return fail(ctx, MUMS_E_INVALID, "sharded restart pending (mums_shard_restart_plan / _apply)");
    *count = ctx->P;
    return MUMS_OK;
}

int mums_probe_copy(mums_ctx* ctx, uint32_t* buckets, uint64_t* ref_index, uint64_t capacity) {
    if (check_ctx(ctx)) return MUMS_E_INVALID;
    if (ctx->stage_done < MUMS_STAGE_SEEDS) return fail(ctx, MUMS_E_INVALID, "no seed stage run");
    if (ctx->shard && ctx->merge_chunked)
        return fail(ctx, MUMS_E_UNSUPPORTED, "probe export after a chunked shard merge");
    if (ctx->shard && ctx->shard_restart_pending)
        return fail(ctx, MUMS_E_INVALID, "sharded restart pending (mums_shard_restart_plan / _apply)");
    if (capacity < ctx->P) return fail(ctx, MUMS_E_INVALID, "output buffer too small");
    if (!ctx->packed_path) return fail(ctx, MUMS_E_UNSUPPORTED, "probe export needs the packed-record path");
    if (ctx->P && (!ctx->probe_info || !ctx->sorted_rec))
        return fail(ctx, MUMS_E_UNSUPPORTED, "probe export after a chunked run (> 2^32 seed-mers)");
    const uint64_t P = ctx->P, N = ctx->N;
    if (P == 0) return MUMS_OK;
    HIPCHK(hipSetDevice(ctx->device));
    std::vector<uint64_t> info(P), rec(N);
    std::vector<uint32_t> bkt(P), ids(P);
    HIPCHK(hipMemcpy(info.data(), ctx->probe_info, P * 8, hipMemcpyDeviceToHost));
    HIPCHK(hipMemcpy(rec.data(), ctx->sorted_rec, N * 8, hipMemcpyDeviceToHost));
    HIPCHK(hipMemcpy(bkt.data(), ctx->sorted_buckets, P * 4, hipMemcpyDeviceToHost));
    HIPCHK(hipMemcpy(ids.data(), ctx->sorted_ids, P * 4, hipMemcpyDeviceToHost));
    std::vector<uint32_t> bucket_of_probe(P);
    for (uint64_t i = 0; i < P; ++i) bucket_of_probe[ids[i]] = bkt[i];
    for (uint64_t k = 0; k < P; ++k) {
        const uint64_t h = (uint32_t)info[k], gs = info[k] >> 32;
        uint64_t mn = ~0ull;
        const uint64_t imask = (1ull << ctx->rec_ib) - 1;
        for (uint64_t i = h; i < h + gs && i < N; ++i) mn = std::min<uint64_t>(mn, rec[i] & imask);
        if (buckets) buckets[k] = bucket_of_probe[k];
        if (ref_index) ref_index[k] = mn;
    }
    return MUMS_OK;
}



namespace {

int shard_seeds_done(mums_ctx* ctx, bool pending_ok = false) {
    if (check_ctx(ctx)) return MUMS_E_INVALID;
    if (!ctx->shard) return fail(ctx, MUMS_E_INVALID, "not a sharded context (mums_shard_layout)");
    if (ctx->stage_done < MUMS_STAGE_SEEDS) return fail(ctx, MUMS_E_INVALID, "no sharded seed stage run");
    if (ctx->shard_restart_pending && !pending_ok)
        return fail(ctx, MUMS_E_INVALID, "sharded restart pending (mums_shard_restart_plan / _apply)");
    return MUMS_OK;
}

int sort_row_keys(mums_ctx* ctx, uint32_t* keys, uint64_t P, int bits, hipStream_t st) {
    uint32_t* kB = (uint32_t*)ctx->rowtmp.p + (P + 64);
    uint32_t* iA = kB + (P + 64);
    uint32_t* iB = iA + (P + 64);
    HIPCHK(ctx->radix_tmp.ensure(radix_tmp_bytes(P + 1)));
    int out = 0;
    HIPCHK(radix_sort<uint32_t>(keys, nullptr, P, bits, kB, iA, keys, iB, ctx->radix_tmp.p, &out, st));
    ctx->sorted_buckets = out ? keys : kB;
    ctx->sorted_ids = out ? iB : iA;
    return MUMS_OK;
}

int enum_count_check(mums_ctx* ctx, hipStream_t st) {
    uint32_t err = 0;
    HIPCHK(hipMemcpyAsync(&err, &ctx->counters.as<DevCounters>()->err, 4, hipMemcpyDeviceToHost, st));
    HIPCHK(hipStreamSynchronize(st));
    if (err & 64u)
        return fail(ctx, MUMS_E_UNSUPPORTED, "enumeration tolerance: a seed group with more than 2^31 AddHashEntry calls");
    return MUMS_OK;
}

int enum_row_offsets(mums_ctx* ctx, const uint32_t* ncalls, uint32_t* off, uint64_t n, uint64_t* total, hipStream_t st) {
    DevCounters* dc = ctx->counters.as<DevCounters>();
    *total = 0;
    HIPCHK(hipMemcpyAsync(off, ncalls, n * 4, hipMemcpyDeviceToDevice, st));
    HIPCHK(exclusive_scan_u32(off, n, ctx->tmp.p, &dc->nprobes, st));
    HIPCHK(launch_sum_u64(ncalls, n, &dc->row_total, st));
// ... 1609 lines not shown
```

### libmems_amd/csrc/mums_internal.h

```cpp
#pragma once

#include <hip/hip_runtime.h>
#include <stdint.h>
#include <stdlib.h>

#include <vector>

#include "restart_plan.h"

namespace mums {

constexpr int kMaxG = 64;
constexpr int kRepeatLimit = 1000;
constexpr int kBlock = 256;
#ifndef MUMS_SEED_TILE
#define MUMS_SEED_TILE 4096
#endif
constexpr int kSeedTile = MUMS_SEED_TILE;
#ifndef MUMS_SEG_TILE
#define MUMS_SEG_TILE 4096
#endif
constexpr int kSegTile = MUMS_SEG_TILE;
constexpr int kLocalIPT = 16;
constexpr int kMaxMsdBits = 11;
// ... 121 lines not shown
__device__ __forceinline__ int genome_of(const GenomeTable& gt, uint64_t i) {
    int g = 0;
    #pragma unroll 1
    for (int k = 1; k < gt.G; ++k) g += (i >= gt.base[k]) ? 1 : 0;
    return g;
}

__host__ __device__ inline uint64_t packed_words(uint64_t n) { return (2 * n) / 32 + (((2 * n) % 32) ? 1 : 0) + 2; }

hipError_t launch_seed_pack(const SeedSpec& ss, const GenomeTable& gt, const char* const* d_ascii,
                            uint32_t* d_packed, int mode, bool key64, void* d_ckey, int msd_bits,
                            uint32_t* d_hist, uint32_t ntiles, uint32_t* d_err, hipStream_t st);
hipError_t launch_seed_scatter(const SeedSpec& ss, const GenomeTable& gt, const uint32_t* d_packed, int msd_bits,
                               const uint32_t* d_hist_scanned, uint32_t ntiles, uint64_t* d_rec, hipStream_t st,
                               uint8_t* d_side = nullptr, int side_bits = 0);
hipError_t launch_seed_scatter_chunk(const SeedSpec& ss, const GenomeTable& gt, const uint32_t* d_packed, int msd_bits,
                                     const uint32_t* d_hist_slice, uint32_t ntiles, uint32_t dlo, uint32_t nbc,
                                     uint64_t* d_rec, hipStream_t st, const uint64_t* d_cbase = nullptr, int mb = 0,
                                     uint8_t* d_side = nullptr, int side_bits = 0);
size_t msd_split_tmp_bytes(uint64_t n, int parent_bits);
hipError_t msd_split(const uint64_t* rin, const uint8_t* side, uint64_t* rout, uint64_t n, int parent_bits, int S,
                     const uint32_t* bstart_in, uint32_t* bstart_out, void* d_tmp, hipStream_t st);
hipError_t launch_keys_of_genome(const SeedSpec& ss, const uint32_t* d_words, uint64_t m, uint64_t* d_out,
                                 hipStream_t st, bool ref_form = true);

size_t scan_tmp_bytes(uint64_t n);
hipError_t exclusive_scan_u32(uint32_t* d_data, uint64_t n, void* d_tmp, uint32_t* d_total, hipStream_t st);
hipError_t launch_sum_u64(const uint32_t* d_data, uint64_t n, unsigned long long* d_total, hipStream_t st);

size_t radix_tmp_bytes(uint64_t n);
template <typename K>
hipError_t radix_sort(const K* keys_in, const uint32_t* vals_in, uint64_t n, int bits,
                      K* kA, uint32_t* vA, K* kB, uint32_t* vB, void* d_tmp, int* out_buf,
                      hipStream_t st, hipEvent_t* ev_ds = nullptr);

uint64_t seg_tiles_upper(uint64_t n, int msd_bits, uint32_t tile = kSegTile);
size_t seg_tmp_bytes(uint64_t n, int msd_bits);
hipError_t launch_regroup(const uint64_t* src, uint64_t* dst, const uint64_t* d_chunks, uint32_t nchunks, uint64_t n,
                          hipStream_t st);
hipError_t seg_bucket_starts(const uint32_t* d_hist_scanned, uint32_t T, int msd_bits, uint64_t n, uint32_t* bstart,
                             hipStream_t st);
hipError_t build_seg_tiles_from_starts(const uint32_t* bstart, int msd_bits, uint64_t n, SegTile* d_tiles,
                                       uint32_t* d_ntiles, void* d_tmp, hipStream_t st, uint32_t tile = kSegTile);
hipError_t build_seg_tiles(const uint32_t* d_hist_scanned, uint32_t T, int msd_bits, uint64_t n, SegTile* d_tiles,
                           uint32_t* d_ntiles, uint32_t* d_bstart, void* d_tmp, hipStream_t st);
hipError_t seg_radix_sort(uint64_t* recA, uint64_t* recB, uint64_t n, int key_bits, const SegTile* d_tiles,
                          uint64_t ntiles_ub, void* d_tmp, int* out_buf, hipStream_t st,
                          hipEvent_t* ev_ds = nullptr);
size_t onesweep_tmp_bytes(uint64_t n, int msd_bits, int key_bits);
hipError_t seg_onesweep_sort(uint64_t* recA, uint64_t* recB, uint64_t n, int key_bits, int msd_bits,
                             const uint32_t* d_bstart, void* d_tmp, uint32_t* d_err, int* out_buf, hipStream_t st,
                             hipEvent_t* ev_ds = nullptr, int key_shift = 32, bool mask_parity = false,
                             bool key_runs = false, const uint32_t* hist_in = nullptr,
                             const uint64_t* gsrc = nullptr, uint32_t* gout = nullptr);
size_t seg_parity_fix_tmp_bytes(uint64_t n);
hipError_t seg_parity_fix(uint64_t* rec, uint64_t* scratch, uint64_t n, int key_bits, int msd_bits,
                          const uint32_t* d_bstart, void* d_tmp, uint32_t* d_err, hipStream_t st, int key_shift = 32);
int seg_onesweep_launches(int key_bits);
bool seg_wide_sort_enabled();
int seg_wide_passes(int key_bits);
size_t onesweep_wide_tmp_bytes(uint64_t n, int msd_bits, int key_bits);
hipError_t seg_onesweep_sort_wide(uint64_t* recA, uint64_t* recB, uint64_t n, int key_bits, int msd_bits,
                                  const uint32_t* d_bstart, void* d_tmp, uint32_t* d_err, int* out_buf,
                                  hipStream_t st, hipEvent_t* ev_ds, int key_shift = 32);

uint64_t group_slot_count(uint64_t ntiles);
uint64_t group_blocks(uint64_t ntiles, bool packed);
template <int MG, typename View>
hipError_t launch_probe_tiles(View v, const SegTile* tiles, uint64_t ntiles, uint64_t N, const GenomeTable& gt,
                              const MatchParams& mp, int L, uint32_t* tile_count, uint64_t* slot_info,
                              uint32_t* slot_bucket, void* counters, hipStream_t st);
hipError_t launch_probe_compact(uint64_t nblocks, const uint32_t* tile_count, const uint32_t* tile_off,
                                const uint64_t* slot_info, const uint32_t* slot_bucket, uint64_t* probe_info,
                                uint32_t* probe_bucket, hipStream_t st, bool packed);
hipError_t launch_bucket_records(const uint32_t* b, uint64_t P, uint64_t* rec, hipStream_t st);
hipError_t launch_bucket_split(const uint64_t* rec, uint64_t P, uint32_t* b, uint32_t* ids, hipStream_t st);
template <int MG, typename View>
hipError_t launch_materialize(View v, const uint64_t* probe_info, uint64_t P, const GenomeTable& gt,
                              const MatchParams& mp, int L, int64_t* rows, hipStream_t st, uint64_t* lkey = nullptr,
                              uint32_t* fsk = nullptr, uint32_t* lhash = nullptr, int32_t* rows32 = nullptr);
hipError_t launch_row_buckets(const int64_t* rows, uint64_t P, int G, uint32_t table_size, const uint32_t* d_bounds,
                              uint32_t nranks, uint32_t* out, hipStream_t st);
hipError_t launch_gather_rows(const int64_t* src, const uint32_t* perm, uint64_t P, int G, int64_t* dst,
                              hipStream_t st);
hipError_t launch_rec_pairs(const uint64_t* rec, uint64_t n, const uint32_t* d_bst, uint32_t nb, uint32_t kfirst,
                            int kb_rec, uint64_t* key, uint32_t* idx, hipStream_t st);
hipError_t launch_rec_pairs33(const uint64_t* rec, uint64_t n, const uint32_t* d_bst, uint32_t nb, uint32_t kfirst,
                              int kb_rec, uint64_t* key, uint64_t* idx, hipStream_t st);
hipError_t launch_chain_dest(const uint32_t* fk, uint64_t nch, const uint32_t* pdest, uint32_t* cdest, hipStream_t st);
hipError_t launch_inverse_perm(const uint32_t* perm, uint64_t n, uint32_t* inv, hipStream_t st);
hipError_t launch_chain_tags(const uint32_t* chain_of, const uint32_t* perm, const uint32_t* sdest, uint64_t P,
                             const uint32_t* cinv, const uint32_t* cstart, uint32_t* tags, hipStream_t st);
hipError_t launch_chain_entries_out(const int64_t* pool, const uint32_t* fk, const uint32_t* cperm,
                                    const uint32_t* scdest, uint64_t nch, int G, const uint32_t* pinv,
                                    const uint32_t* rstart, int64_t* eout, uint32_t* fout, hipStream_t st);
hipError_t launch_kept_dest(const int64_t* rows, uint64_t P, int G, const uint32_t* chain_of, const uint32_t* cinv,
                            const uint2* thr, const uint32_t* fk, const uint32_t* pdest, uint32_t nranks, uint32_t* dest,
                            hipStream_t st);
hipError_t launch_dest_first(const uint32_t* sdest, uint64_t P, uint32_t* first, hipStream_t st);
hipError_t launch_entry_first(const uint32_t* scdest, uint64_t nch, const uint32_t* rcount, const uint32_t* perm,
                              const uint32_t* sdest, uint64_t K, const uint32_t* chain_of, const uint32_t* cinv,
                              const uint32_t* rstart, uint32_t* efirst, hipStream_t st);
hipError_t launch_flat_tiles(uint64_t N, SegTile* d_tiles, hipStream_t st);

hipError_t launch_bucket_ranges(const uint32_t* sb, uint64_t P, uint32_t* bstart, uint32_t* bend, uint32_t* d_max,
                                hipStream_t st);
template <int MG, typename View>
hipError_t launch_replay_kept(View v, const GenomeTable& gt, const MatchParams& mp, int L, uint64_t P,
                              const int64_t* pool, const uint32_t* chain_of, const uint32_t* fk, uint32_t nch,
                              void* d_tmp, void* d_radix_tmp, void* d_scan_tmp, uint32_t lds_cap, uint32_t* tsize,
                              void* ctr, uint64_t* dbg, hipStream_t st, uint64_t* mlog, uint32_t** tbl_out,
                              const uint32_t** base_out, void* (*alloc)(void*, size_t), void* alloc_ctx,
                              const uint32_t* jl = nullptr);
}
struct mums_ctx;
namespace mums {
hipStream_t ctx_stream(mums_ctx* ctx);
int ctx_device(mums_ctx* ctx);
int ctx_table_genomes(mums_ctx* ctx, uint32_t* table_size, uint32_t* genomes);
uint32_t ctx_repeat_tol(mums_ctx* ctx);
bool ctx_merge_chunked(mums_ctx* ctx);
bool ctx_tie_all(mums_ctx* ctx);
bool ctx_pcompat(mums_ctx* ctx);
int ctx_compat_layout(mums_ctx* ctx, uint32_t* first, uint32_t* nown, std::vector<uint64_t>* lens);
int ctx_compat_rank_find(mums_ctx* ctx, const char* const* d_ascii, const uint64_t* lens, int G, uint32_t rank,
                         uint32_t ranks, int stage);
int ctx_compat_rank_export(mums_ctx* ctx, uint64_t* bucket_counts, int64_t* d_rows, uint64_t* M);
int ctx_compat_rank_merge(mums_ctx* ctx, const int64_t* d_rows, uint32_t W, const uint64_t* counts, uint32_t nb);

// ... 245 lines not shown
```

### libmems_amd/csrc/radix_seg.hip

```cpp
#include <algorithm>
#include <cstdio>
#include <cstdlib>
#include <cstring>
#include <type_traits>
#include <vector>

#include "mums_internal.h"

namespace mums {

namespace {

constexpr int kTile = kSegTile;
constexpr int kRounds = kTile / kBlock;
constexpr int kWaves = kBlock / 64;
constexpr int kDigits = 256;
#ifndef MUMS_SORT_BLOCK
#define MUMS_SORT_BLOCK 768
#endif
#ifndef MUMS_SORT_TILE
#define MUMS_SORT_TILE 9216
#endif
#ifndef MUMS_SORT_NT
#define MUMS_SORT_NT 0
// ... 324 lines not shown
                        }
                    }
                }
            } else {
                #pragma unroll
                for (int u = 0; u < kGhistBatch; ++u) {
                    if (q0 + u * kBlock + tid >= d.count) break;
                    const uint64_t key = kk[u] >> key_shift;
                    for (int p = 0; p < nh; ++p) atomicAdd(&h[p][(uint32_t)(key >> (8 * p)) & 0xFFu], 1u);
                }
            }
        }
    }
    __syncthreads();
    if (cur_b != 0xFFFFFFFFu)
        for (int p = 0; p < nh; ++p) {
            const uint32_t v = h[p][tid];
            if (v) atomicAdd(&ghist[((uint64_t)cur_b * npass + p) * kDigits + tid], v);
        }
}

__global__ __launch_bounds__(kBlock) void seg_dbase_kernel(const uint32_t* __restrict__ ghist,
                                                           const uint32_t* __restrict__ bstart, int npass,
                                                           uint32_t* __restrict__ dbase, int pass) {
    __shared__ uint32_t s_w[kWaves];
    const uint64_t bp = pass < 0 ? (uint64_t)blockIdx.x : (uint64_t)blockIdx.x * npass + pass;
    const uint32_t b = (uint32_t)(bp / npass);
    const int lane = threadIdx.x & 63, wv = threadIdx.x >> 6;
    const uint32_t v = ghist[bp * kDigits + threadIdx.x];
    uint32_t inc = v;
    #pragma unroll
    for (int dd = 1; dd < 64; dd <<= 1) {
        const uint32_t x = __shfl_up(inc, dd, 64);
        if (lane >= dd) inc += x;
    }
    if (lane == 63) s_w[wv] = inc;
    __syncthreads();
    uint32_t pre = 0;
    #pragma unroll
    for (int w = 0; w < kWaves; ++w) pre += (w < wv) ? s_w[w] : 0u;
    dbase[bp * kDigits + threadIdx.x] = bstart[b] + pre + inc - v;
}

template <int kIPT>
__device__ __forceinline__ void onesweep_load(const uint64_t* __restrict__ rin, const SegTile& d, uint32_t q0, int lane,
                                              uint64_t (&key)[kIPT]) {
    #pragma unroll
    for (int r = 0; r < kIPT; ++r) {
        const uint32_t q = q0 + r * 64 + lane;
        key[r] = q < d.count ? rin[d.start + q] : 0ull;
    }
}

template <int OB, int kIPT, bool kAlias = false, bool kLate = false, bool kGath = false, bool kHi = false>
__global__ __launch_bounds__(OB) __attribute__((amdgpu_waves_per_eu(OB == 768 ? 6 : 1)))
void seg_onesweep_kernel(const uint64_t* __restrict__ rin,
                                                          uint64_t* __restrict__ rout,
                                                          const SegTile* __restrict__ tiles, uint32_t nclaims,
                                                          int shift, int pass, int npass,
                                                          const uint32_t* __restrict__ dbase, uint32_t* status,
                                                          uint32_t* tile_counter, uint32_t* err,
                                                          uint32_t* __restrict__ ghist_next,
                                                          const uint32_t* __restrict__ xq,
                                                          const uint64_t* __restrict__ gsrc = nullptr,
                                                          uint32_t* __restrict__ gout = nullptr,
                                                          const uint4* __restrict__ xd = nullptr) {
    constexpr int kT = kIPT * OB;
    constexpr bool late = MUMS_OS_LATEPUB || kLate;
    constexpr int kW = OB / 64;
    static_assert(OB >= kDigits, "one thread per digit");
    static_assert(!kAlias || kW * kDigits * 4 <= kT * 8, "counts fit in the exchange buffer");
    __shared__ uint64_t srec[kT];
    __shared__ uint32_t wcnt_own[kAlias ? 1 : kW][kDigits];
    uint32_t (*wcnt)[kDigits] = kAlias ? reinterpret_cast<uint32_t (*)[kDigits]>(srec) : wcnt_own;
    __shared__ uint32_t lstart[kDigits];
    __shared__ uint32_t gofs[kDigits];
    __shared__ uint32_t s_w[kDigits / 64];
    __shared__ uint32_t s_tile;
    __shared__ uint32_t hcnt[kDigits];
    __shared__ uint32_t hnext[kDigits];
    __shared__ uint4 s_desc;
    __shared__ uint32_t s_far;
    const int tid = threadIdx.x, lane = tid & 63, wv = tid >> 6;
#if MUMS_OS_STATS
    unsigned long long ts[8] = {0, 0, 0, 0, 0, 0, 0, 0};
#endif
    OS_STAMP(0);
    if (tid == 0) {
        if (xq) {
            uint32_t tt = 0xFFFFFFFFu;
            const uint32_t x = blockIdx.x & 7u;
            for (uint32_t a = 0; a < 8; ++a) {
                const uint32_t q = (x + a) & 7u;
                const uint32_t qo = xq[8 + q], ql = xq[q];
                const uint32_t cc = atomicAdd(tile_counter + q, 1u);
                if (cc < ql) {
                    if (xd) {
                        const uint4 dd = xd[qo + cc];
                        s_desc = dd;
                        tt = dd.x;
                    } else {
                        tt = xq[32 + qo + cc];
                    }
                    break;
                }
            }
            s_tile = tt;
        } else {
            s_tile = atomicAdd(tile_counter, 1u);
        }
    }
    for (int i = tid; i < kW * kDigits; i += OB) (&wcnt[0][0])[i] = 0;
    if (tid < kDigits) { hcnt[tid] = 0; hnext[tid] = 0; }
    if (tid == 0) s_far = 0;
    __syncthreads();
    const uint32_t c = __builtin_amdgcn_readfirstlane(s_tile);
    if (xq ? c == 0xFFFFFFFFu : c >= nclaims) return;
#if MUMS_OS_CTILES
    const SegTile d = tiles[c];
    const uint32_t t = __builtin_amdgcn_readfirstlane(d.order);
#else
    const uint32_t t = xq ? c : __builtin_amdgcn_readfirstlane(tiles[c].order);
    SegTile d{};
    if (xd) {
        const uint4 dd = s_desc;
        d.start = __builtin_amdgcn_readfirstlane(dd.y);
        d.count = __builtin_amdgcn_readfirstlane(dd.z & 0xFFFFu);
        d.bucket = __builtin_amdgcn_readfirstlane(dd.z >> 16);
        d.tb = __builtin_amdgcn_readfirstlane(dd.w);
    } else {
        d = tiles[t];
    }
#endif
    if (d.count == 0) return;
    OS_STAMP(1);
    const uint32_t q0 = wv * (kT / kW);
    auto qof = [&](int r) -> uint32_t { return q0 + (uint32_t)r * 64u + (uint32_t)lane; };
    auto digit = [&](uint64_t k) -> uint32_t {
        if constexpr (kHi) return ((uint32_t)(k >> 32) >> (shift - 32)) & 0xFFu;
        else return (uint32_t)(k >> shift) & 0xFFu;
    };
    auto digit_next = [&](uint64_t k) -> uint32_t {
        if constexpr (kHi) return ((uint32_t)(k >> 32) >> (shift - 24)) & 0xFFu;
        else return (uint32_t)(k >> (shift + 8)) & 0xFFu;
    };
    const uint32_t bb = __builtin_amdgcn_readfirstlane(dbase[((uint64_t)d.bucket * npass + pass) * kDigits]);
    static_assert((uint64_t)kT * 8 < (1ull << 32), "32-bit byte offsets inside a tile");
    const bool full = d.count == (uint32_t)kT;
    const uint32_t pad = (uint32_t)kT - d.count;
    uint64_t key[kIPT];
    uint32_t rank[kIPT];
    const char* tin = reinterpret_cast<const char*>(rin + d.start);
    auto loads = [&](auto full_c) {
        #pragma unroll
        for (int r = 0; r < kIPT; ++r) {
            const uint32_t q = qof(r);
            const bool in = decltype(full_c)::value || q < d.count;
#if MUMS_SORT_NT & 1
            key[r] = in ? __builtin_nontemporal_load(reinterpret_cast<const uint64_t*>(tin + q * 8u)) : ~0ull;
#else
            key[r] = in ? *reinterpret_cast<const uint64_t*>(tin + q * 8u) : ~0ull;
#endif
        }
    };
    if (full) loads(std::true_type{});
    else loads(std::false_type{});
    if constexpr (!late) {
        #pragma unroll
        for (int r = 0; r < kIPT; ++r)
            atomicAdd(&hcnt[digit(key[r])], 1u);
        __syncthreads();
        OS_STAMP(2);
        if (d.tb != 0 && tid < kDigits)
            __hip_atomic_store(status + (uint64_t)t * kDigits + tid,
                               kFlagAgg | (hcnt[tid] - (tid == kDigits - 1 ? pad : 0u)), __ATOMIC_RELAXED,
                               __HIP_MEMORY_SCOPE_AGENT);
    }
    if (ghist_next) {
        #pragma unroll
        for (int r = 0; r < kIPT; ++r)
            atomicAdd(&hnext[digit_next(key[r])], 1u);
    }
    #pragma unroll
    for (int r = 0; r < kIPT; ++r) {
        uint32_t tot;
        const uint32_t rk = wave_match_rank<8>(digit(key[r]), &tot);
        const uint32_t old = wcnt[wv][digit(key[r])];
        if (rk == 0) wcnt[wv][digit(key[r])] = old + tot;
        rank[r] = old + rk;
    }
    __syncthreads();
    OS_STAMP(3);
    uint32_t v = 0, acc = 0;
    if (tid < kDigits) {
        const int dgt = tid;
        #pragma unroll
        for (int w = 0; w < kW; ++w) { const uint32_t x = wcnt[w][dgt]; wcnt[w][dgt] = acc; acc += x; }
        if (dgt == kDigits - 1) acc -= pad;
        uint32_t* st = status + (uint64_t)t * kDigits + dgt;
        if (late && d.tb != 0) __hip_atomic_store(st, kFlagAgg | acc, __ATOMIC_RELAXED, __HIP_MEMORY_SCOPE_AGENT);
        uint32_t prefix = 0;
        if (d.tb == 0) {
            __hip_atomic_store(st, kFlagInc | acc, __ATOMIC_RELAXED, __HIP_MEMORY_SCOPE_AGENT);
        } else {
            const int64_t tfirst = (int64_t)t - (int64_t)d.tb;
            int64_t j = (int64_t)t - 1;
            uint32_t spins = 0;
            bool done = false;
            while (!done) {
                uint32_t sv[kLookback];
// ... 24 lines not shown
                               __HIP_MEMORY_SCOPE_AGENT);
        }
        const uint32_t rel = dbase[((uint64_t)d.bucket * npass + pass) * kDigits + dgt] - bb + prefix;
        gofs[dgt] = rel;
        if (rel >= (1u << 29) - (uint32_t)kT) s_far = 1u;
        v = acc;
        #pragma unroll
        for (int dd = 1; dd < 64; dd <<= 1) {
            const uint32_t x = __shfl_up(v, dd, 64);
            if (lane >= dd) v += x;
        }
        if (lane == 63) s_w[wv] = v;
    }
    __syncthreads();
    OS_STAMP(4);
    if (tid < kDigits) {
        uint32_t wpre = 0;
        #pragma unroll
        for (int w = 0; w < kDigits / 64; ++w) wpre += (w < wv) ? s_w[w] : 0u;
        lstart[tid] = wpre + v - acc;
#if MUMS_OS_FUSED
        const uint32_t ls = wpre + v - acc;
        #pragma unroll
        for (int w = 0; w < kW; ++w) wcnt[w][tid] += ls;
        gofs[tid] -= ls;
#endif
    }
    __syncthreads();
    if constexpr (kAlias) {
        #pragma unroll
        for (int r = 0; r < kIPT; ++r) {
#if MUMS_OS_FUSED
            rank[r] += wcnt[wv][digit(key[r])];
#else
            rank[r] += lstart[digit(key[r])] + wcnt[wv][digit(key[r])];
#endif
        }
        __syncthreads();
        #pragma unroll
        for (int r = 0; r < kIPT; ++r) srec[rank[r]] = key[r];
    } else {
    #pragma unroll
    for (int r = 0; r < kIPT; ++r) {
#if MUMS_OS_FUSED
        srec[wcnt[wv][digit(key[r])] + rank[r]] = key[r];
#else
        srec[lstart[digit(key[r])] + wcnt[wv][digit(key[r])] + rank[r]] = key[r];
#endif
    }
    }
    __syncthreads();
    OS_STAMP(5);
    uint64_t* bout = rout + bb;
    uint32_t* bgout = kGath ? gout + bb : nullptr;
    auto stores = [&](auto full_c, auto far_c) {
        constexpr bool kFar = decltype(far_c)::value;
        #pragma unroll
        for (int r = 0; r < kIPT; ++r) {
            const uint32_t sidx = tid + r * OB;
            if (decltype(full_c)::value || sidx < d.count) {
                const uint64_t k = srec[sidx];
                const uint32_t sd = digit(k);
#if MUMS_OS_FUSED
                const uint32_t o = gofs[sd] + sidx;
#else
                const uint32_t o = gofs[sd] + (sidx - lstart[sd]);
#endif
                if constexpr (kGath) {
                    const uint32_t gv = (uint32_t)gsrc[(uint32_t)k];
                    if constexpr (kFar) bgout[o] = gv;
                    else *reinterpret_cast<uint32_t*>(reinterpret_cast<char*>(bgout) + o * 4u) = gv;
                } else {
                    uint64_t* op = kFar ? bout + o
                                        : reinterpret_cast<uint64_t*>(reinterpret_cast<char*>(bout) + o * 8u);
#if MUMS_SORT_NT & 2
                    __builtin_nontemporal_store(k, op);
#else
                    *op = k;
#endif
                }
            }
        }
    };
    if (s_far) stores(std::false_type{}, std::true_type{});
    else if (full) stores(std::true_type{}, std::false_type{});
    else stores(std::false_type{}, std::false_type{});
    if (ghist_next && tid < kDigits) {
        const uint32_t c = hnext[tid] - (tid == kDigits - 1 ? pad : 0u);
        if (c) atomicAdd(&ghist_next[((uint64_t)d.bucket * npass + pass + 1) * kDigits + tid], c);
    }
#if MUMS_OS_STATS
    OS_STAMP(6);
    __builtin_amdgcn_s_waitcnt(0);
    OS_STAMP(7);
    if (tid == 0) {
        unsigned long long* o = g_os_stats + (uint64_t)t * 10;
        for (int k = 0; k < 8; ++k) o[k] = ts[k];
        o[8] = blockIdx.x;
        o[9] = 1;
    }
#endif
}

template <int OB, int kIPT>
__global__ __launch_bounds__(OB) __attribute__((amdgpu_waves_per_eu(4))) void seg_onesweep_persist_kernel(const uint64_t* __restrict__ rin,
                                                                  uint64_t* __restrict__ rout,
                                                                  const SegTile* __restrict__ tiles,
                                                                  uint32_t nclaims, int shift, int pass, int npass,
                                                                  const uint32_t* __restrict__ dbase,
                                                                  uint32_t* status, uint32_t* tile_counter,
                                                                  uint32_t* err) {
    constexpr int kT = kIPT * OB;
    constexpr int kW = OB / 64;
    static_assert(OB >= kDigits, "one thread per digit");
    __shared__ uint64_t srec[kT];
    __shared__ uint32_t wcnt[kW][kDigits];
    __shared__ uint32_t lstart[kDigits];
    __shared__ uint32_t gofs[kDigits];
    __shared__ uint32_t s_w[kDigits / 64];
    __shared__ uint32_t s_tile[2];
    __shared__ uint32_t hcnt[kDigits];
    const int tid = threadIdx.x, lane = tid & 63, wv = tid >> 6;
    const uint32_t q0 = wv * (kT / kW);
    if (tid == 0) s_tile[0] = atomicAdd(tile_counter, 1u);
// ... 517 lines not shown
    const size_t b = (ub * kDigits * (uint64_t)npass + 2 * nb * npass * kDigits + 256 + 64) * 4 +
                     2 * (ub * sizeof(SegTile) + 256) + seg_build_tmp_bytes(nb) + segfix_cap(n) * 4 +
                     256;
    return seg_wide_sort_enabled() ? std::max(b, onesweep_wide_tmp_bytes(n, msd_bits, key_bits)) : b;
}

static hipError_t launch_segfix(uint64_t* rec, uint64_t* scratch, uint64_t n, const SfMode& md, const uint32_t* d_bstart,
                                int nb, uint32_t* big_count, void* d_list, uint32_t* d_err, hipStream_t st) {
    const uint64_t tiles = (n + kSfTile - 1) / kSfTile;
    const uint32_t cap = (uint32_t)segfix_cap(n);
    uint32_t* big_list = (uint32_t*)d_list;
    unsigned long long* dbg = nullptr;
    const bool stats = getenv("MUMS_DEV_SEGFIX_STATS") != nullptr;
    if (stats) {
        dbg = (unsigned long long*)(big_count + 2);
        (void)hipMemsetAsync(dbg, 0, 32, st);
    }
    hipLaunchKernelGGL(segfix_tile_kernel, dim3((unsigned)tiles), dim3(kBlock), 0, st, rec, (uint32_t)n, md, d_bstart,
                       nb, big_list, big_count, cap, d_err, seg_segfix_force_big(), dbg);
    hipLaunchKernelGGL(segfix_big_kernel, dim3(256), dim3(kBlock), 0, st, rec, scratch, (uint32_t)n, md, d_bstart, nb,
                       big_list, big_count, cap);
    if (stats) {
        uint32_t hc[2] = {0, 0};
        unsigned long long hd[4] = {0, 0, 0, 0};
        (void)hipMemcpyAsync(hc, big_count, 8, hipMemcpyDeviceToHost, st);
        (void)hipMemcpyAsync(hd, dbg, 32, hipMemcpyDeviceToHost, st);
        (void)hipStreamSynchronize(st);
        fprintf(stderr, "segfix: n=%llu tiles=%llu dmask=%u big=%u forced=%u cyc/block load=%.0f flags=%.0f jobs=%llu job_recs=%llu\n",
                (unsigned long long)n, (unsigned long long)tiles, md.dmask, hc[0], hc[1], hd[0] / (double)tiles,
                hd[1] / (double)tiles, hd[2], hd[3]);
    }
    return hipGetLastError();
}

size_t seg_parity_fix_tmp_bytes(uint64_t n) { return 256 + segfix_cap(n) * 4 + 256; }

hipError_t seg_parity_fix(uint64_t* rec, uint64_t* scratch, uint64_t n, int key_bits, int msd_bits,
                          const uint32_t* d_bstart, void* d_tmp, uint32_t* d_err, hipStream_t st, int key_shift) {
    if (n == 0 || key_bits < 2) return hipSuccess;
    SfMode md;
    md.dshift = key_shift;
    md.dmask = 1u;
    md.pshift = key_shift + 1;
    md.pmask = (1ull << (key_bits - 1)) - 1;
    uint32_t* big_count = (uint32_t*)d_tmp;
    hipError_t e = hipMemsetAsync(big_count, 0, 64, st);
    if (e != hipSuccess) return e;
    return launch_segfix(rec, scratch, n, md, d_bstart, 1 << msd_bits, big_count, (char*)d_tmp + 256, d_err, st);
}

hipError_t seg_onesweep_sort(uint64_t* recA, uint64_t* recB, uint64_t n, int key_bits, int msd_bits,
                             const uint32_t* d_bstart, void* d_tmp, uint32_t* d_err, int* out_buf, hipStream_t st,
                             hipEvent_t* ev_ds, int key_shift, bool mask_parity, bool key_runs,
                             const uint32_t* hist_in, const uint64_t* gsrc, uint32_t* gout) {
    const int nkd = (key_bits + 7) / 8;
    const bool segfix = nkd >= 2 && seg_segfix_enabled();
    const int npass = segfix ? nkd - 1 : nkd;
    const int digit_shift = key_shift;
    if (segfix) key_shift += 8;
    *out_buf = npass % 2;
    if (n == 0 || npass == 0) return hipSuccess;
    if (nkd > 4) return hipErrorInvalidValue;
    const uint64_t nb = 1ull << msd_bits;
    const int tile = os_tile();
    const uint64_t ub = seg_tiles_upper(n, msd_bits, tile);
    uint32_t* status = (uint32_t*)d_tmp;
    uint32_t* ghist = status + ub_status(ub, npass);
    uint32_t* dbase = ghist + nb * npass * kDigits;
    uint32_t* counters = dbase + nb * npass * kDigits;
    const size_t zero_bytes = ((uint64_t)(counters - status) + 256) * 4;
    SegTile* stiles = (SegTile*)((char*)d_tmp + ((zero_bytes + 255) & ~(size_t)255));
    SegTile* ctiles = (SegTile*)((char*)stiles + ((ub * sizeof(SegTile) + 255) & ~(size_t)255));
    void* btmp = (void*)((char*)ctiles + ((ub * sizeof(SegTile) + 255) & ~(size_t)255));
    hipError_t e = hipMemsetAsync(status, 0, zero_bytes, st);
    if (e != hipSuccess) return e;
    e = build_seg_tiles_from_starts(d_bstart, msd_bits, n, stiles, counters + 32, btmp, st, tile);
    if (e != hipSuccess) return e;
#if MUMS_OS_CTILES
    hipLaunchKernelGGL(claim_tiles_kernel, dim3((unsigned)((ub + 255) / 256)), dim3(256), 0, st, stiles, ub, ctiles);
    const SegTile* otiles = ctiles;
    uint32_t* xq = nullptr;
#else
    const SegTile* otiles = stiles;
    uint32_t* xq = (os_xcd() && nb >= 8 && !MUMS_SORT_PERSIST) ? (uint32_t*)ctiles : nullptr;
    uint4* xqd = xq ? (uint4*)(((uintptr_t)(xq + 32 + ub) + 15) & ~(uintptr_t)15) : nullptr;
    const uint4* xd = os_xd() ? xqd : nullptr;
    if (xq)
        hipLaunchKernelGGL(xcd_order_kernel, dim3((unsigned)((ub + 255) / 256)), dim3(256), 0, st,
                           (const uint32_t*)btmp, (int)nb, ub, stiles, xq, xqd);
#endif
    const unsigned gblocks = (unsigned)((ub + kGhistTilesPerBlock - 1) / kGhistTilesPerBlock);
    const bool nexthist = MUMS_OS_NEXTHIST && !MUMS_SORT_PERSIST;
    if (hist_in && nb == 1 && !segfix && !nexthist) {
        e = hipMemcpyAsync(ghist, hist_in, (size_t)npass * kDigits * 4, hipMemcpyDeviceToDevice, st);
        if (e != hipSuccess) return e;
    } else {
        hipLaunchKernelGGL(seg_ghist_kernel, dim3(gblocks), dim3(kBlock), 0, st, recA, stiles, ub, npass, ghist,
                           key_shift, nexthist ? 1 : npass, key_runs ? 1 : 0);
    }
    if (nexthist)
        hipLaunchKernelGGL(seg_dbase_kernel, dim3((unsigned)nb), dim3(kBlock), 0, st, ghist, d_bstart, npass, dbase,
                           0);
    else
        hipLaunchKernelGGL(seg_dbase_kernel, dim3((unsigned)(nb * npass)), dim3(kBlock), 0, st, ghist, d_bstart,
                           npass, dbase, -1);
#if MUMS_SORT_PERSIST
    uint64_t persist_grid = 0;
    {
        int dev = 0, cus = 0, per = 0;
        (void)hipGetDevice(&dev);
        (void)hipDeviceGetAttribute(&cus, hipDeviceAttributeMultiprocessorCount, dev);
        (void)hipOccupancyMaxActiveBlocksPerMultiprocessor(
            &per, (const void*)seg_onesweep_persist_kernel<kSortBlock, kSortTile / kSortBlock>, kSortBlock, 0);
        persist_grid = (uint64_t)std::max(cus, 1) * (uint64_t)std::max(per, 1);
    }
#endif
#if MUMS_OS_STATS
    unsigned long long* os_dev = nullptr;
    (void)hipMalloc(&os_dev, ub * 80);
    (void)hipMemsetAsync(os_dev, 0, ub * 80, st);
    (void)hipMemcpyToSymbol(HIP_SYMBOL(g_os_stats), &os_dev, sizeof(os_dev), 0, hipMemcpyHostToDevice);
#endif
    uint64_t* src = recA;
    uint64_t* dst = recB;
    for (int p = 0; p < npass; ++p) {
        if (ev_ds) (void)hipEventRecord(ev_ds[2 * p], st);
#if MUMS_SORT_PERSIST
        hipLaunchKernelGGL((seg_onesweep_persist_kernel<kSortBlock, kSortTile / kSortBlock>),
                           dim3((unsigned)std::min<uint64_t>(ub, persist_grid)), dim3(kSortBlock), 0, st, src, dst,
                           stiles, (uint32_t)ub, key_shift + 8 * p, p, npass, dbase,
                           status + (uint64_t)p * ub * kDigits, counters + p, d_err);
#else
        {
            uint32_t* gn = (nexthist && p + 1 < npass) ? ghist : (uint32_t*)nullptr;
            uint32_t* sp = status + (uint64_t)p * ub * kDigits;
            const int sh = key_shift + 8 * p;
            uint32_t* tc = xq ? counters + 128 + 8 * p : counters + p;
#define MUMS_OS_LAUNCH1(OB, IPT, AL, HI)                                                                     \
    hipLaunchKernelGGL((seg_onesweep_kernel<OB, IPT, AL, false, false, HI>), dim3((unsigned)ub), dim3(OB), 0, st, src, \
                       dst, otiles, (uint32_t)ub, sh, p, npass, dbase, sp, tc, d_err, gn, xq, nullptr, nullptr, xd)
#define MUMS_OS_LAUNCH(OB, IPT, AL)                     \
    do {                                                \
        if (sh >= 32) MUMS_OS_LAUNCH1(OB, IPT, AL, true); \
        else MUMS_OS_LAUNCH1(OB, IPT, AL, false);       \
    } while (0)
            if (key_runs && gout && p + 1 == npass) {
                hipLaunchKernelGGL((seg_onesweep_kernel<kSortBlock, kSortTile / kSortBlock, true, true, true>),
                                   dim3((unsigned)ub), dim3(kSortBlock), 0, st, src, dst, otiles, (uint32_t)ub, sh, p,
                                   npass, dbase, sp, tc, d_err, gn, xq, gsrc, gout, xd);
            } else if (key_runs) {
                hipLaunchKernelGGL((seg_onesweep_kernel<kSortBlock, kSortTile / kSortBlock, true, true>),
                                   dim3((unsigned)ub), dim3(kSortBlock), 0, st, src, dst, otiles, (uint32_t)ub, sh, p,
                                   npass, dbase, sp, tc, d_err, gn, xq, nullptr, nullptr, xd);
            } else
            switch (os_variant()) {
            case 1: MUMS_OS_LAUNCH(512, 16, true); break;
            case 2: MUMS_OS_LAUNCH(512, 12, true); break;
            case 3: MUMS_OS_LAUNCH(384, 16, true); break;
            case 4: MUMS_OS_LAUNCH(256, 16, true); break;
            case 5: MUMS_OS_LAUNCH(512, 8, true); break;
            case 6: MUMS_OS_LAUNCH(1024, 8, true); break;
            case 7: MUMS_OS_LAUNCH(512, 16, false); break;
            case 8: MUMS_OS_LAUNCH(640, 14, true); break;
            default: MUMS_OS_LAUNCH(kSortBlock, kSortTile / kSortBlock, true); break;
            }
#undef MUMS_OS_LAUNCH
#undef MUMS_OS_LAUNCH1
        }
#endif
        e = hipGetLastError();
        if (e != hipSuccess) return e;
#if MUMS_OS_STATS
        {
            (void)hipStreamSynchronize(st);
            std::vector<unsigned long long> hs(ub * 10);
            (void)hipMemcpy(hs.data(), os_dev, ub * 80, hipMemcpyDeviceToHost);
            double ph[7] = {0, 0, 0, 0, 0, 0, 0}, tot = 0;
            unsigned long long lo[8], hi[8];
            double busy[8] = {0, 0, 0, 0, 0, 0, 0, 0};
            for (int x = 0; x < 8; ++x) { lo[x] = ~0ull; hi[x] = 0; }
            uint64_t nt = 0;
            for (uint64_t i = 0; i < ub; ++i) {
                const unsigned long long* o = &hs[i * 10];
                if (!o[9]) continue;
                ++nt;
                for (int k = 1; k < 8; ++k) ph[k - 1] += (double)(o[k] - o[k - 1]);
                tot += (double)(o[7] - o[0]);
                const int x = (int)(o[8] & 7);
                lo[x] = std::min(lo[x], o[0]);
                hi[x] = std::max(hi[x], o[7]);
                busy[x] += (double)(o[7] - o[0]);
            }
            const double d = nt ? (double)nt * 100.0 : 1.0;
            double bs = 0, wl = 0;
            for (int x = 0; x < 8; ++x)
                if (hi[x] > lo[x]) { bs += busy[x] / (double)(hi[x] - lo[x]); wl = std::max(wl, (double)(hi[x] - lo[x])); }
            fprintf(stderr, "os_stats n=%llu pass=%d tiles=%llu us/tile: claim %.2f load+count %.2f rank %.2f lookback %.2f "
                    "lstart+exch %.2f stores %.2f drain %.2f | tile %.2f us, XCD wall %.1f us, busy block slots %.1f\n",
                    (unsigned long long)n, p, (unsigned long long)nt, ph[0] / d, ph[1] / d, ph[2] / d, ph[3] / d,
                    ph[4] / d, ph[5] / d, ph[6] / d, tot / d, wl / 100.0, bs);
            (void)hipMemset(os_dev, 0, ub * 80);
        }
#endif
        if (nexthist && p + 1 < npass)
            hipLaunchKernelGGL(seg_dbase_kernel, dim3((unsigned)nb), dim3(kBlock), 0, st, ghist, d_bstart, npass,
                               dbase, p + 1);
        if (ev_ds) (void)hipEventRecord(ev_ds[2 * p + 1], st);
        uint64_t* t = src;
        src = dst;
        dst = t;
    }
#if MUMS_OS_STATS
    (void)hipStreamSynchronize(st);
    (void)hipFree(os_dev);
#endif
    if (segfix) {
        if (ev_ds) (void)hipEventRecord(ev_ds[2 * npass], st);
        SfMode md;
        md.dshift = mask_parity ? digit_shift + 1 : digit_shift;
        md.dmask = mask_parity ? 0x7Fu : 0xFFu;
        md.pshift = digit_shift + 8;
        md.pmask = (1ull << (key_bits - 8)) - 1;
        e = launch_segfix(src, dst, n, md, d_bstart, (int)nb, counters + 48, (char*)btmp + seg_build_tmp_bytes(nb),
                          d_err, st);
        if (e != hipSuccess) return e;
        if (ev_ds) (void)hipEventRecord(ev_ds[2 * npass + 1], st);
    }
    return hipSuccess;
}

hipError_t seg_radix_sort(uint64_t* recA, uint64_t* recB, uint64_t n, int key_bits, const SegTile* d_tiles,
                          uint64_t ntiles_ub, void* d_tmp, int* out_buf, hipStream_t st, hipEvent_t* ev_ds) {
    const int passes = (key_bits + 7) / 8;
    *out_buf = passes % 2;
    if (n == 0 || passes == 0) return hipSuccess;
    const uint64_t h = ntiles_ub * kDigits;
    uint32_t* hist = (uint32_t*)d_tmp;
    void* stmp = (void*)(hist + h + 64);
    uint64_t* src = recA;
    uint64_t* dst = recB;
    for (int p = 0; p < passes; ++p) {
        const int shift = 32 + 8 * p;
        hipLaunchKernelGGL(seg_upsweep, dim3((unsigned)ntiles_ub), dim3(kBlock), 0, st, src, d_tiles, shift, hist);
        hipError_t e = exclusive_scan_u32(hist, h, stmp, nullptr, st);
        if (e != hipSuccess) return e;
        if (ev_ds) (void)hipEventRecord(ev_ds[2 * p], st);
        hipLaunchKernelGGL(seg_downsweep, dim3((unsigned)ntiles_ub), dim3(kBlock), 0, st, src, d_tiles, shift, hist,
                           dst);
        e = hipGetLastError();
        if (e != hipSuccess) return e;
        if (ev_ds) (void)hipEventRecord(ev_ds[2 * p + 1], st);
        uint64_t* t = src;
        src = dst;
        dst = t;
    }
    return hipSuccess;
}

}
```

### libmems_amd/csrc/replay.hip

```cpp
#include <algorithm>
#include <cstdio>
#include <cstdlib>
#include <vector>

#include "match_device.h"
#include "seed_device.h"

namespace mums {

namespace {

__device__ __forceinline__ void log_insert(uint64_t* mlog, DevCounters* ctr, uint32_t probe, uint32_t cid) {
    if (mlog) mlog[atomicAdd(&ctr->log_n, 1ull)] = ((uint64_t)probe << 32) | cid;
}

template <int RB>
__device__ __forceinline__ int block_first_true(bool pred, int* red) {
    const int lane = threadIdx.x & 63, wv = threadIdx.x >> 6;
    const uint64_t b = __ballot(pred);
    if (lane == 0) red[wv] = b ? wv * 64 + (__ffsll((long long)b) - 1) : RB;
    __syncthreads();
    int r = red[0];
    #pragma unroll
    for (int w = 1; w < RB / 64; ++w) r = min(r, red[w]);
// ... 44 lines not shown
    uint32_t first = 0, len = t;
    while (len > 0) {
        const uint32_t half = len >> 1, mid = first + half;
        const uint4 X = tb[mid];
        int r = slot_cmp(X, vmask, vs, vl, vcid);
        if (r == 2) r = full(X.x) ? 1 : 0;
        if (r) {
            first = mid + 1;
            len = len - half - 1;
        } else {
            len = half;
        }
    }
    return first;
}

template <int MG>
__device__ __forceinline__ uint32_t block_key(const Mhe<MG>& m, int G, const uint32_t* __restrict__ bkey,
                                              uint32_t cid) {
    if constexpr (MG > 32) {
        return bkey[cid];
    } else {
        uint32_t k = 0;
        #pragma unroll
        for (int g = 0; g < MG; ++g) k |= (g < G && m.s[g] != 0) ? (1u << g) : 0u;
        return __builtin_bitreverse32(k);
    }
}

__global__ __launch_bounds__(kBlock) void chain_bmask_kernel(const int64_t* __restrict__ pool, uint32_t nch, int G,
                                                             uint64_t* __restrict__ out) {
    const uint32_t c = blockIdx.x * kBlock + threadIdx.x;
    if (c >= nch) return;
    const int64_t* e = pool + (uint64_t)c * (uint64_t)(G + 2);
    uint64_t m = 0;
    for (int g = 0; g < G; ++g) m |= e[2 + g] != 0 ? (1ull << g) : 0ull;
    out[c] = __builtin_bitreverse64(m);
}

__global__ __launch_bounds__(kBlock) void dense_step_kernel(const uint64_t* __restrict__ skey, uint32_t n,
                                                            uint32_t* __restrict__ step) {
    const uint32_t i = blockIdx.x * kBlock + threadIdx.x;
    if (i < n) step[i] = (i + 1 < n && skey[i + 1] != skey[i]) ? 1u : 0u;
}

__global__ __launch_bounds__(kBlock) void dense_scatter_kernel(const uint32_t* __restrict__ ord,
                                                               const uint32_t* __restrict__ rank, uint32_t n,
                                                               uint32_t* __restrict__ bkey) {
    const uint32_t i = blockIdx.x * kBlock + threadIdx.x;
    if (i < n) bkey[ord[i]] = rank[i];
}

__global__ __launch_bounds__(kBlock) void chain_keys_kernel(const int64_t* __restrict__ pool, uint32_t nch, int G,
                                                            uint32_t table_size, double inv_t,
                                                            const uint32_t* __restrict__ bkey,
                                                            uint64_t* __restrict__ key_s, uint64_t* __restrict__ key_b) {
    const uint32_t c = blockIdx.x * kBlock + threadIdx.x;
    if (c >= nch) return;
    const int64_t* e = pool + (uint64_t)c * (uint64_t)(G + 2);
    uint32_t m = 0;
    int64_t s0 = 0;
    for (int g = G - 1; g >= 0; --g) {
        const int64_t sg = e[2 + g];
        if (sg != 0) { m |= g < 32 ? 1u << g : 0u; s0 = sg; }
    }
    key_s[c] = (uint64_t)s0;
    key_b[c] = ((uint64_t)bucket_of_fast(e[1], table_size, inv_t) << 32) | (bkey ? bkey[c] : __builtin_bitreverse32(m));
}

__global__ __launch_bounds__(kBlock) void gather_gkey_kernel(const uint64_t* __restrict__ key_b,
                                                             const uint32_t* __restrict__ idx, uint32_t n,
                                                             int low_shift, int kb, uint64_t* __restrict__ dst) {
    const uint32_t i = blockIdx.x * kBlock + threadIdx.x;
    if (i >= n) return;
    const uint64_t b = key_b[idx[i]];
    dst[i] = ((b >> 32) << kb) | (uint64_t)((uint32_t)b >> low_shift);
}

__global__ __launch_bounds__(kBlock) void chain_next_kernel(const uint32_t* __restrict__ ord,
                                                            const uint64_t* __restrict__ key_s,
                                                            const uint64_t* __restrict__ key_b, uint32_t nch,
                                                            uint32_t* __restrict__ next_s,
                                                            uint32_t* __restrict__ rank) {
    const uint32_t i = blockIdx.x * kBlock + threadIdx.x;
    if (i >= nch) return;
    const uint32_t c = ord[i];
    const uint64_t g = key_b[c], sc = key_s[c];
    uint64_t nx = ~0ull;
    bool tie = false;
    if (i + 1 < nch) {
        const uint32_t d = ord[i + 1];
        if (key_b[d] == g) nx = key_s[d];
        tie = nx == sc;
    }
    if (i > 0) {
        const uint32_t d = ord[i - 1];
        if (key_b[d] == g && key_s[d] == sc) { nx = sc; tie = true; }
    }
    next_s[c] = nx > 0xFFFFFFFFull ? 0xFFFFFFFFu : (uint32_t)nx;
    rank[c] = i | (tie ? 0x80000000u : 0u);
}

__global__ __launch_bounds__(kBlock) void chain_sb_kernel(const int64_t* __restrict__ pool, uint32_t nch, int G,
                                                          const uint32_t* __restrict__ rank,
                                                          const uint32_t* __restrict__ next_s,
                                                          uint4* __restrict__ chain_sb) {
    const uint32_t c = blockIdx.x * kBlock + threadIdx.x;
// ... 1206 lines not shown
        if ((want >> i) & 1u) {
            if (o < cap) {
                kept[o] = keys[i];
                kcid[o] = cids[i];
            }
            ++o;
        }
}

template <int MG, typename View>
__global__ __launch_bounds__(kBlock) void kept_summary_kernel(View v, GenomeTable gt, int L,
                                                              const uint64_t* __restrict__ skey, uint32_t Kc,
                                                              const uint32_t* __restrict__ scid,
                                                              const uint32_t* __restrict__ fk,
                                                              const uint4* __restrict__ chain_sb,
                                                              const uint32_t* __restrict__ bkey,
                                                              uint4* __restrict__ summ, uint4* __restrict__ summ_b) {
    const uint32_t i = blockIdx.x * kBlock + threadIdx.x;
    if (i >= Kc) return;
    const uint32_t k = (uint32_t)skey[i];
    Mhe<MG> Q;
    load_probe<MG>(v, k, gt.G, L, Q);
    const uint32_t cid = scid[i];
    const uint4 cs = chain_sb[cid];
    const bool first = fk[cid] == k;
    summ[i] = make_uint4(block_key<MG>(Q, gt.G, bkey, cid), (uint32_t)start_at(Q, first_start(Q)), cid,
                         first ? 0x80000000u : 0x40000000u);
    summ_b[i] = make_uint4(cs.x, cs.y, cs.z, k);
}

__global__ __launch_bounds__(kBlock) void kept_ranges_kernel(const uint64_t* __restrict__ skey, uint32_t Kc,
                                                             uint32_t* __restrict__ cbeg, uint32_t* __restrict__ cend,
                                                             uint64_t P, DevCounters* __restrict__ ctr) {
    const uint32_t i = blockIdx.x * kBlock + threadIdx.x;
    if (i == 0) atomicAdd(&ctr->collisions, (unsigned long long)(P - Kc));
    if (i >= Kc) return;
    const uint32_t b = (uint32_t)(skey[i] >> 32);
    if (i == 0 || (uint32_t)(skey[i - 1] >> 32) != b) cbeg[b] = i;
    if (i + 1 == Kc || (uint32_t)(skey[i + 1] >> 32) != b) cend[b] = i + 1;
}

static hipError_t chain_order(const int64_t* pool, uint32_t nch, const GenomeTable& gt, const MatchParams& mp,
                              uint64_t* key_s, uint64_t* key_b, uint64_t* key_g, uint64_t* kA, uint64_t* kB,
                              uint32_t* vA, uint32_t* vB, uint32_t* step, uint32_t* bkey_buf, void* d_radix_tmp,
                              void* d_scan_tmp, uint32_t* next_s, uint32_t* rank, const uint32_t** bkey_out,
                              hipStream_t st) {
    const unsigned cgrid = (nch + kBlock - 1) / kBlock;
    hipError_t e = hipSuccess;
    const uint32_t* bkey = block_keys(pool, nch, gt.G, key_g, kA, vA, kB, vB, step, bkey_buf, d_radix_tmp,
                                      d_scan_tmp, st, &e);
    if (e != hipSuccess) return e;
    *bkey_out = bkey;
    hipLaunchKernelGGL(chain_keys_kernel, dim3(cgrid), dim3(kBlock), 0, st, pool, nch, gt.G, mp.table_size,
                       1.0 / (double)mp.table_size, bkey, key_s, key_b);
    if ((e = hipGetLastError()) != hipSuccess) return e;
    int buf = 0;
    if ((e = radix_sort<uint64_t>(key_s, nullptr, nch, 32, kA, vA, kB, vB, d_radix_tmp, &buf, st)) != hipSuccess)
        return e;
    const uint32_t* ord1 = buf ? vB : vA;
    int tb = 1;
    while (tb < 32 && ((uint64_t)1 << tb) < (uint64_t)mp.table_size) ++tb;
    int kb = 32, low_shift = 0;
    if (!bkey) {
        kb = gt.G;
        low_shift = 32 - gt.G;
    } else {
        kb = 1;
        while (kb < 32 && ((uint64_t)1 << kb) < (uint64_t)nch) ++kb;
    }
    hipLaunchKernelGGL(gather_gkey_kernel, dim3(cgrid), dim3(kBlock), 0, st, key_b, ord1, nch, low_shift, kb, key_g);
    uint32_t* vin = buf ? vB : vA;
    uint32_t* vout = buf ? vA : vB;
    int buf2 = 0;
    if ((e = radix_sort<uint64_t>(key_g, vin, nch, kb + tb, kA, vout, kB, vin, d_radix_tmp, &buf2, st)) != hipSuccess)
        return e;
    const uint32_t* ord = buf2 ? vin : vout;
    hipLaunchKernelGGL(chain_next_kernel, dim3(cgrid), dim3(kBlock), 0, st, ord, key_s, key_b, nch, next_s, rank);
    return hipGetLastError();
}

template <int MG, typename View>
hipError_t launch_replay_kept(View v, const GenomeTable& gt, const MatchParams& mp, int L, uint64_t P,
                              const int64_t* pool, const uint32_t* chain_of, const uint32_t* fk, uint32_t nch,
                              void* d_tmp, void* d_radix_tmp, void* d_scan_tmp, uint32_t lds_cap, uint32_t* tsize,
                              void* ctr, uint64_t* dbg, hipStream_t st, uint64_t* mlog, uint32_t** tbl_out,
                              const uint32_t** base_out, void* (*alloc)(void*, size_t), void* alloc_ctx,
                              const uint32_t* jl) {
    char* p = (char*)d_tmp;
    auto carve = [&](size_t bytes) {
        char* r = p;
        p += (bytes + 255) & ~(size_t)255;
        return (void*)r;
    };
    uint64_t* key_s = (uint64_t*)carve((size_t)nch * 8);
    uint64_t* key_b = (uint64_t*)carve((size_t)nch * 8);
    uint64_t* key_g = (uint64_t*)carve((size_t)nch * 8);
    uint64_t* kA = (uint64_t*)carve((size_t)nch * 8);
    uint64_t* kB = (uint64_t*)carve((size_t)nch * 8);
    uint32_t* vA = (uint32_t*)carve((size_t)nch * 4);
    uint32_t* vB = (uint32_t*)carve((size_t)nch * 4);
    uint32_t* next_s = (uint32_t*)carve((size_t)nch * 4);
    uint32_t* rank = (uint32_t*)carve((size_t)nch * 4);
    uint4* chain_sb = (uint4*)carve((size_t)nch * 16);
    uint32_t* bkey_buf = (uint32_t*)carve((size_t)nch * 4);
    const uint64_t nblk = (P + kBlock * kKeepIPT - 1) / (kBlock * kKeepIPT);
    unsigned int* nkept = (unsigned int*)carve(64);
    uint4* ckeep = (uint4*)carve((size_t)nch * 16);
// ... 169 lines not shown
```

Before: 40.80 billion seed-mers/s.

## Fuse bucket histogram into probe compaction and sort 32-bit bucket keys directly

Result: faster. 41.81 billion seed-mers/s, median of 6 (+2.5%).

```diff
diff --git a/libmems_amd/csrc/groups.hip b/libmems_amd/csrc/groups.hip
--- a/libmems_amd/csrc/groups.hip
+++ b/libmems_amd/csrc/groups.hip
@@ -164,7 +164,7 @@
                                                                 uint64_t* __restrict__ slot_info,
                                                                 uint32_t* __restrict__ slot_bucket,
                                                                 DevCounters* __restrict__ ctr,
-                                                                double inv_table) {
+                                                                uint64_t bucket_rcp) {
     constexpr int kGRounds = kGSubRounds;
     constexpr int kWaves = kBlock / 64;
     __shared__ uint64_t srec[kGSub];
@@ -272,7 +272,7 @@
     const TileRecViewT<IB> v{(lds_u64*)srec, rec, tile0, cnt};
     const bool fast = kFastOnly || (mp.repeat_tol == 0 && mp.enum_tol == 1);
     const uint64_t want_mn = mp.masked ? mp.seq_mask : 0ull;
-    const double inv_t = inv_table;
+    const uint64_t inv_t = bucket_rcp;
     const uint64_t sb = (uint64_t)blockIdx.x * kSubSlots;
     uint32_t nrep = 0, base = 0, buf = 0;
     for (uint32_t c = 0; c < H; c += kBlock) {
@@ -356,6 +356,65 @@
     }
 }
 
+constexpr int kCompactWgs = 16;
+constexpr int kCompactIPT = 4;
+
+__global__ __launch_bounds__(kBlock) void probe_compact_hist_kernel(const uint32_t* __restrict__ tile_count,
+                                                                    const uint32_t* __restrict__ tile_off,
+                                                                    const uint64_t* __restrict__ slot_info,
+                                                                    const uint32_t* __restrict__ slot_bucket,
+                                                                    uint64_t* __restrict__ probe_info,
+                                                                    uint32_t* __restrict__ probe_bucket,
+                                                                    uint32_t slots_per_block, uint32_t nwg, int npass,
+                                                                    uint32_t* __restrict__ hist) {
+    __shared__ uint32_t s_off[kCompactWgs + 1];
+    __shared__ uint32_t s_h[4][256];
+    const uint32_t w0 = blockIdx.x * (uint32_t)kCompactWgs;
+    const uint32_t nw = nwg - w0 < (uint32_t)kCompactWgs ? nwg - w0 : (uint32_t)kCompactWgs;
+    const uint32_t o0 = tile_off[w0];
+    if (threadIdx.x <= (uint32_t)kCompactWgs) {
+        const uint32_t w = threadIdx.x < nw ? threadIdx.x : nw - 1;
+        s_off[threadIdx.x] = tile_off[w0 + w] - o0 + (threadIdx.x < nw ? 0u : tile_count[w0 + w]);
+    }
+    for (int i = threadIdx.x; i < 4 * 256; i += kBlock) (&s_h[0][0])[i] = 0;
+    __syncthreads();
+    const uint32_t total = s_off[kCompactWgs];
+    for (uint32_t j0 = 0; j0 < total; j0 += kBlock * kCompactIPT) {
+        uint64_t info[kCompactIPT];
+        uint32_t bkt[kCompactIPT];
+        #pragma unroll
+        for (int u = 0; u < kCompactIPT; ++u) {
+            const uint32_t j = j0 + u * kBlock + threadIdx.x;
+            uint32_t m = 0;
+            #pragma unroll
+            for (int s = kCompactWgs / 2; s > 0; s >>= 1) m += s_off[m + s] <= j ? (uint32_t)s : 0u;
+            const uint64_t src = (uint64_t)(w0 + m) * slots_per_block + (j - s_off[m]);
+            info[u] = j < total ? slot_info[src] : 0ull;
+            bkt[u] = j < total ? slot_bucket[src] : 0u;
+        }
+        #pragma unroll
+        for (int u = 0; u < kCompactIPT; ++u) {
+            const uint32_t j = j0 + u * kBlock + threadIdx.x;
+            const bool valid = j < total;
+            if (valid) {
+                probe_info[(uint64_t)o0 + j] = info[u];
+                probe_bucket[(uint64_t)o0 + j] = bkt[u];
+            }
+            for (int p = 0; p < npass; ++p) {
+                const uint32_t dg = (bkt[u] >> (8 * p)) & 0xFFu;
+                uint32_t tot;
+                const uint32_t rk = wave_match_rank<8>(dg, valid, &tot);
+                if (valid && rk == 0) atomicAdd(&s_h[p][dg], tot);
+            }
+        }
+    }
+    __syncthreads();
+    for (int p = 0; p < npass; ++p) {
+        const uint32_t c = s_h[p][threadIdx.x];
+        if (c) atomicAdd(&hist[p * 256 + threadIdx.x], c);
+    }
+}
+
 __global__ void flat_tiles_kernel(uint64_t N, uint64_t nt, SegTile* __restrict__ tiles) {
     const uint64_t t = (uint64_t)blockIdx.x * blockDim.x + threadIdx.x;
     if (t >= nt) return;
@@ -475,7 +534,7 @@
 }
 
 __global__ __launch_bounds__(kBlock) void row_bucket_kernel(const int64_t* __restrict__ rows, uint64_t P, int G,
-                                                            uint32_t table_size, double inv_t,
+                                                            uint32_t table_size, uint64_t inv_t,
                                                             const uint32_t* __restrict__ bounds, uint32_t nranks,
                                                             uint32_t* __restrict__ out) {
     const uint64_t k = (uint64_t)blockIdx.x * kBlock + threadIdx.x;
@@ -509,21 +568,6 @@
         const uint64_t e = e0 + (uint64_t)i * kBlock;
         if (e < n) dst[e] = x[i];
     }
-}
-
-__global__ __launch_bounds__(kBlock) void bucket_rec_kernel(const uint32_t* __restrict__ b, uint64_t P,
-                                                            uint64_t* __restrict__ rec) {
-    const uint64_t k = (uint64_t)blockIdx.x * kBlock + threadIdx.x;
-    if (k < P) rec[k] = ((uint64_t)b[k] << 32) | k;
-}
-
-__global__ __launch_bounds__(kBlock) void bucket_split_kernel(const uint64_t* __restrict__ rec, uint64_t P,
-                                                              uint32_t* __restrict__ b, uint32_t* __restrict__ ids) {
-    const uint64_t k = (uint64_t)blockIdx.x * kBlock + threadIdx.x;
-    if (k >= P) return;
-    const uint64_t r = rec[k];
-    b[k] = (uint32_t)(r >> 32);
-    ids[k] = (uint32_t)r;
 }
 
 __global__ __launch_bounds__(kBlock) void chain_dest_kernel(const uint32_t* __restrict__ fk, uint64_t nch,
@@ -703,19 +747,6 @@
     return hipGetLastError();
 }
 
-hipError_t launch_bucket_records(const uint32_t* b, uint64_t P, uint64_t* rec, hipStream_t st) {
-    if (P == 0) return hipSuccess;
-    hipLaunchKernelGGL(bucket_rec_kernel, dim3((unsigned)((P + kBlock - 1) / kBlock)), dim3(kBlock), 0, st, b, P, rec);
-    return hipGetLastError();
-}
-
-hipError_t launch_bucket_split(const uint64_t* rec, uint64_t P, uint32_t* b, uint32_t* ids, hipStream_t st) {
-    if (P == 0) return hipSuccess;
-    hipLaunchKernelGGL(bucket_split_kernel, dim3((unsigned)((P + kBlock - 1) / kBlock)), dim3(kBlock), 0, st, rec, P, b,
-                       ids);
-    return hipGetLastError();
-}
-
 uint64_t group_slot_count(uint64_t ntiles) { return ntiles * kSlots; }
 uint64_t group_blocks(uint64_t ntiles, bool packed) { return packed ? ntiles * kGSplit : ntiles; }
 
@@ -737,7 +768,7 @@
                               uint32_t nranks, uint32_t* out, hipStream_t st) {
     if (P == 0) return hipSuccess;
     hipLaunchKernelGGL(row_bucket_kernel, dim3((unsigned)((P + kBlock - 1) / kBlock)), dim3(kBlock), 0, st, rows, P, G,
-                       table_size, 1.0 / (double)table_size, d_bounds, nranks, out);
+                       table_size, bucket_recip(table_size), d_bounds, nranks, out);
     return hipGetLastError();
 }
 
@@ -765,7 +796,7 @@
     if (ntiles == 0) return hipSuccess;
     if constexpr (RecIB<View>::value > 0) {
         const bool fast = mp.repeat_tol == 0 && mp.enum_tol == 1;
-        const double inv_t = 1.0 / (double)mp.table_size;
+        const uint64_t inv_t = bucket_recip(mp.table_size);
         if (RecIB<View>::value == 32 && gt.gl_n > 0 && fast && !getenv("MUMS_DEV_PROBE_GENERAL"))
             hipLaunchKernelGGL((probe_tile_rec_kernel<MG, RecIB<View>::value, true, true>),
                                dim3((unsigned)(ntiles * kGSplit)), dim3(kBlock), 0, st, v.rec, tiles, gt, mp, L,
@@ -786,8 +817,17 @@
 
 hipError_t launch_probe_compact(uint64_t nblocks, const uint32_t* tile_count, const uint32_t* tile_off,
                                 const uint64_t* slot_info, const uint32_t* slot_bucket, uint64_t* probe_info,
-                                uint32_t* probe_bucket, hipStream_t st, bool packed) {
+                                uint32_t* probe_bucket, hipStream_t st, bool packed, uint32_t* bucket_hist,
+                                int hist_passes) {
     if (nblocks == 0) return hipSuccess;
+    if (bucket_hist) {
+        static_assert(kBlock == 256, "one histogram bin per thread");
+        if (hist_passes < 1 || hist_passes > 4 || nblocks > 0xFFFFFFFFull) return hipErrorInvalidValue;
+        hipLaunchKernelGGL(probe_compact_hist_kernel, dim3((unsigned)((nblocks + kCompactWgs - 1) / kCompactWgs)),
+                           dim3(kBlock), 0, st, tile_count, tile_off, slot_info, slot_bucket, probe_info, probe_bucket,
+                           (uint32_t)(packed ? kSubSlots : kSlots), (uint32_t)nblocks, hist_passes, bucket_hist);
+        return hipGetLastError();
+    }
     hipLaunchKernelGGL(probe_compact_kernel, dim3((unsigned)nblocks), dim3(kBlock), 0, st, tile_count, tile_off,
                        slot_info, slot_bucket, probe_info, probe_bucket, (uint32_t)(packed ? kSubSlots : kSlots));
     return hipGetLastError();
diff --git a/libmems_amd/csrc/match_device.h b/libmems_amd/csrc/match_device.h
--- a/libmems_amd/csrc/match_device.h
+++ b/libmems_amd/csrc/match_device.h
@@ -1,5 +1,6 @@
 #pragma once
 
+#include <cstring>
 #include <type_traits>
 
 #include "mums_internal.h"
@@ -263,14 +264,37 @@
     return probe_offset_batch<MG, View>(r, v, h, end, gt, mp, L, offset, gsize);
 }
 
-__device__ __forceinline__ uint32_t bucket_of_fast(int64_t offset, uint32_t table_size, double inv_t) {
+#ifndef MUMS_BUCKET_INT
+#define MUMS_BUCKET_INT 0
+#endif
+#if !MUMS_BUCKET_INT
+inline uint64_t bucket_recip(uint32_t table_size) {
+    const double inv = 1.0 / (double)table_size;
+    uint64_t b;
+    memcpy(&b, &inv, 8);
+    return b;
+}
+
+__device__ __forceinline__ uint32_t bucket_of_fast(int64_t offset, uint32_t table_size, uint64_t recip) {
     const int64_t T = (int64_t)table_size;
-    const int64_t q = (int64_t)floor((double)offset * inv_t);
+    const int64_t q = (int64_t)floor((double)offset * __longlong_as_double((long long)recip));
     int64_t r = offset - q * T;
     r = r < 0 ? r + T : r;
     r = r >= T ? r - T : r;
     return (uint32_t)r;
 }
+#else
+__host__ __device__ inline uint64_t bucket_recip(uint32_t table_size) { return ~0ull / (uint64_t)table_size; }
+
+__device__ __forceinline__ uint32_t bucket_of_fast(int64_t offset, uint32_t table_size, uint64_t recip) {
+    const uint64_t sign = (uint64_t)(offset >> 63);
+    const uint64_t u = (uint64_t)offset ^ sign;
+    const uint64_t q = __umul64hi(u, recip);
+    uint32_t r = (uint32_t)u - (uint32_t)q * table_size;
+    r = r >= table_size ? r - table_size : r;
+    return sign ? table_size - 1u - r : r;
+}
+#endif
 
 typedef __attribute__((address_space(3))) const uint8_t lds_u8c;
 typedef __attribute__((address_space(3))) const uint32_t lds_u32c;
diff --git a/libmems_amd/csrc/mums_capi.hip b/libmems_amd/csrc/mums_capi.hip
--- a/libmems_amd/csrc/mums_capi.hip
+++ b/libmems_amd/csrc/mums_capi.hip
@@ -112,7 +112,6 @@
     uint32_t nchunks = 0;
     DevBuf cval, ctab;
     DevBuf fsk;
-    DevBuf bst2;
     bool fused_keys = false;
     bool rows_narrow = false;
     DevBuf smlk0, smlkA, smlkB, smlvA, smlvB, smltmp, flen, fs;
@@ -266,10 +265,21 @@
     return hi - lo + 1;
 }
 
+struct BucketHist {
+    uint32_t* d = nullptr;
+    int npass = 0;
+};
+
+int table_bits(uint32_t table_size) {
+    int tbits = 1;
+    while (tbits < 32 && ((uint64_t)1 << tbits) < (uint64_t)table_size) ++tbits;
+    return tbits;
+}
+
 template <int MG, typename View>
 int run_groups(mums_ctx* ctx, View v, const SegTile* tiles, uint64_t ntiles, const MatchParams& mp,
                uint64_t* probe_info, uint32_t* probe_bucket, uint64_t* slot_info, uint32_t* slot_bucket,
-               hipStream_t st) {
+               hipStream_t st, BucketHist bh = BucketHist{}) {
     const bool packed = RecIB<View>::value > 0;
     const uint64_t nb = group_blocks(ntiles, packed);
     uint32_t* counts = ctx->partials.as<uint32_t>();
@@ -281,19 +291,22 @@
     HIPCHK(exclusive_scan_u32(gcounts, nb, ctx->tmp.p, &dc->ngroups, st));
     HIPCHK(hipMemcpyAsync(offs, counts, nb * 4, hipMemcpyDeviceToDevice, st));
     HIPCHK(exclusive_scan_u32(offs, nb, ctx->tmp.p, &dc->nprobes, st));
-    HIPCHK(launch_probe_compact(nb, counts, offs, slot_info, slot_bucket, probe_info, probe_bucket, st, packed));
+    if (bh.d) HIPCHK(hipMemsetAsync(bh.d, 0, (size_t)bh.npass * 256 * 4, st));
+    HIPCHK(launch_probe_compact(nb, counts, offs, slot_info, slot_bucket, probe_info, probe_bucket, st, packed, bh.d,
+                                bh.npass));
     return MUMS_OK;
 }
 
 template <typename View>
 int groups_dispatch(mums_ctx* ctx, View v, const SegTile* tiles, uint64_t ntiles, const MatchParams& mp,
-                    uint64_t* pi, uint32_t* pb, uint64_t* si, uint32_t* sb, hipStream_t st) {
+                    uint64_t* pi, uint32_t* pb, uint64_t* si, uint32_t* sb, hipStream_t st,
+                    BucketHist bh = BucketHist{}) {
     const int G = ctx->gt.G;
-    if (G <= 4) return run_groups<4, View>(ctx, v, tiles, ntiles, mp, pi, pb, si, sb, st);
-    if (G <= 8) return run_groups<8, View>(ctx, v, tiles, ntiles, mp, pi, pb, si, sb, st);
-    if (G <= 16) return run_groups<16, View>(ctx, v, tiles, ntiles, mp, pi, pb, si, sb, st);
-    if (G <= 32) return run_groups<32, View>(ctx, v, tiles, ntiles, mp, pi, pb, si, sb, st);
-    return run_groups<64, View>(ctx, v, tiles, ntiles, mp, pi, pb, si, sb, st);
+    if (G <= 4) return run_groups<4, View>(ctx, v, tiles, ntiles, mp, pi, pb, si, sb, st, bh);
+    if (G <= 8) return run_groups<8, View>(ctx, v, tiles, ntiles, mp, pi, pb, si, sb, st, bh);
+    if (G <= 16) return run_groups<16, View>(ctx, v, tiles, ntiles, mp, pi, pb, si, sb, st, bh);
+    if (G <= 32) return run_groups<32, View>(ctx, v, tiles, ntiles, mp, pi, pb, si, sb, st, bh);
+    return run_groups<64, View>(ctx, v, tiles, ntiles, mp, pi, pb, si, sb, st, bh);
 }
 
 void* devbuf_alloc(void* b, size_t bytes) {
@@ -720,13 +733,15 @@
     uint32_t* idsA;
     uint32_t* idsB;
     uint32_t* slot_bucket;
+    uint32_t* bucket_hist;
 };
 
 int ensure_probe_space(mums_ctx* ctx, uint64_t N, uint64_t ntiles_groups, ProbeSpace* ps) {
     const uint64_t pcap = (N / 2 + 2) & ~1ull;
     const uint64_t nslots = group_slot_count(ntiles_groups);
     HIPCHK(ctx->partials.ensure((3 * group_blocks(ntiles_groups, true) + 128) * 4));
-    HIPCHK(ctx->pbuf.ensure(pcap * (8 + 4 * 4) + nslots * 12 + 256));
+    const uint64_t hist_at = (pcap * (8 + 4 * 4) + nslots * 12 + 255) & ~255ull;
+    HIPCHK(ctx->pbuf.ensure(hist_at + (4 * 256 + 64) * 4 + 256));
     char* pb = (char*)ctx->pbuf.p;
     ps->probe_info = (uint64_t*)pb;
     ps->slot_info = ps->probe_info + pcap;
@@ -735,6 +750,7 @@
     ps->idsA = ps->bucketB + pcap;
     ps->idsB = ps->idsA + pcap;
     ps->slot_bucket = ps->idsB + pcap;
+    ps->bucket_hist = (uint32_t*)(pb + hist_at);
     return MUMS_OK;
 }
 
@@ -821,7 +837,8 @@
 bool wants_tie_order(const mums_ctx* ctx);
 
 int merge_stage(mums_ctx* ctx, uint64_t n, int mb, int key_bits, const MatchParams& mp, const ProbeSpace& ps,
-                hipStream_t st, int ib = 32, uint64_t* rA = nullptr, uint64_t* rB = nullptr) {
+                hipStream_t st, int ib = 32, uint64_t* rA = nullptr, uint64_t* rB = nullptr,
+                BucketHist bh = BucketHist{}) {
     DevCounters* dc = ctx->counters.as<DevCounters>();
     if (!rA) rA = ctx->recA.as<uint64_t>();
     if (!rB) rB = ctx->recB.as<uint64_t>();
@@ -863,12 +880,15 @@
     }
     if (ib == 33)
         return groups_dispatch<RecViewT<33>>(ctx, RecViewT<33>{ctx->sorted_rec}, tiles, ub, mp, ps.probe_info,
-                                             ps.probe_bucket, ps.slot_info, ps.slot_bucket, st);
+                                             ps.probe_bucket, ps.slot_info, ps.slot_bucket, st, bh);
     return groups_dispatch<RecView>(ctx, RecView{ctx->sorted_rec}, tiles, ub, mp, ps.probe_info, ps.probe_bucket,
-                                    ps.slot_info, ps.slot_bucket, st);
-}
-
-int finish_seeds(mums_ctx* ctx, const ProbeSpace& ps, hipStream_t st, bool find_follows = false) {
+                                    ps.slot_info, ps.slot_bucket, st, bh);
+}
+
+constexpr uint64_t kBucketOnesweepMin = 4096;
+
+int finish_seeds(mums_ctx* ctx, const ProbeSpace& ps, hipStream_t st, bool find_follows = false,
+                 BucketHist bh = BucketHist{}) {
     DevCounters* dc = ctx->counters.as<DevCounters>();
     HIPCHK(hipMemcpyAsync(&ctx->hc, dc, sizeof(DevCounters), hipMemcpyDeviceToHost, st));
     HIPCHK(hipStreamSynchronize(st));
@@ -878,8 +898,7 @@
     ctx->P = ctx->hc.nprobes;
     ctx->probe_info = ps.probe_info;
     HIPCHK(hipEventRecord(ctx->ev[EV_GROUPS], st));
-    int tbits = 1;
-    while (tbits < 32 && ((uint64_t)1 << tbits) < (uint64_t)ctx->table_size) ++tbits;
+    const int tbits = table_bits(ctx->table_size);
     const uint64_t P = ctx->P;
     if (find_follows && P > 0 && P <= find_chunk() && !ctx->shard && !getenv("MUMS_DEV_KEEP_BUCKET_ORDER")) {
         ctx->sorted_buckets = nullptr;
@@ -887,19 +906,27 @@
         HIPCHK(hipEventRecord(ctx->ev[EV_BUCKETS], st));
         return MUMS_OK;
     }
-    const bool radix = getenv("MUMS_DEV_BUCKET_ONESWEEP") == nullptr;
-    if (!radix && P >= 4096 && P < (1ull << 30) && ps.slot_info + P <= (const uint64_t*)ps.probe_bucket &&
+    const bool radix = getenv("MUMS_DEV_BUCKET_RADIX") != nullptr;
+    if (!radix && bh.d && bh.npass == (tbits + 7) / 8 && seg_onesweep_launches(tbits) == bh.npass &&
+        P >= kBucketOnesweepMin &&
+        P < (1ull << 30) && ps.slot_info + P <= (const uint64_t*)ps.probe_bucket &&
         ctx->tmp.cap >= onesweep_tmp_bytes(P, 0, tbits)) {
         uint64_t* rA = ps.slot_info;
         uint64_t* rB = (uint64_t*)ps.bucketB;
-        HIPCHK(ctx->bst2.ensure(64));
-        HIPCHK(launch_bucket_records(ps.probe_bucket, P, rA, st));
-        HIPCHK(seg_bucket_starts(nullptr, 0, 0, P, ctx->bst2.as<uint32_t>(), st));
-        int ob = 0;
-        HIPCHK(seg_onesweep_sort(rA, rB, P, tbits, 0, ctx->bst2.as<uint32_t>(), ctx->tmp.p, &dc->err, &ob, st));
-        HIPCHK(launch_bucket_split(ob ? rB : rA, P, ps.probe_bucket, ps.idsB, st));
-        ctx->sorted_buckets = ps.probe_bucket;
-        ctx->sorted_ids = ps.idsB;
+        uint32_t* bst = bh.d + 4 * 256;
+        const bool reads_b = bh.npass == 3;
+        uint32_t* ob = reads_b ? ps.probe_bucket : ps.bucketB;
+        uint32_t* oi = reads_b ? ps.idsB : ps.idsA;
+        HIPCHK(seg_bucket_starts(nullptr, 0, 0, P, bst, st));
+        int obuf = 0;
+        HIPCHK(seg_onesweep_sort(rA, rB, P, tbits, 0, bst, ctx->tmp.p, &dc->err, &obuf, st, nullptr, 32, false, true,
+                                 bh.d, nullptr, nullptr, ps.probe_bucket, ob, oi));
+        uint32_t err = 0;
+        HIPCHK(hipMemcpyAsync(&err, &dc->err, 4, hipMemcpyDeviceToHost, st));
+        HIPCHK(hipStreamSynchronize(st));
+        if (err & 2u) return fail(ctx, MUMS_E_HIP, "sort look-back timed out (internal error)");
+        ctx->sorted_buckets = ob;
+        ctx->sorted_ids = oi;
     } else {
         int pout = 0;
         HIPCHK(radix_sort<uint32_t>(ps.probe_bucket, nullptr, P, tbits, ps.bucketB, ps.idsA, ps.probe_bucket,
@@ -1240,12 +1267,15 @@
     if (prof && !ctx->ev_ds[0])
         for (int i = 0; i < 16; ++i) HIPCHK(hipEventCreate(&ctx->ev_ds[i]));
 
+    BucketHist bh{};
+    if (ctx->packed_path && stage < MUMS_STAGE_ALL && !getenv("MUMS_DEV_BUCKET_RADIX"))
+        bh = BucketHist{ps.bucket_hist, (table_bits(ctx->table_size) + 7) / 8};
     int rc = MUMS_OK;
     if (ctx->packed_path) {
         rc = keys_stage(ctx, gt, T, B, N, ctx->recA.as<uint64_t>(), ctx->mstart.as<uint32_t>(), st, 32, side);
         if (rc) return rc;
         HIPCHK(hipEventRecord(ctx->ev[EV_KEYS], st));
-        rc = merge_stage(ctx, N, B, kbits - B, mp, ps, st);
+        rc = merge_stage(ctx, N, B, kbits - B, mp, ps, st, 32, nullptr, nullptr, bh);
     } else {
         std::vector<const char*> ptrs(G);
         for (int g = 0; g < G; ++g) ptrs[g] = ctx->genomes[g].d_ptr;
@@ -1290,7 +1320,7 @@
                                                      ps.slot_info, ps.slot_bucket, st);
     }
     if (rc) return rc;
-    rc = finish_seeds(ctx, ps, st, stage >= MUMS_STAGE_ALL);
+    rc = finish_seeds(ctx, ps, st, stage >= MUMS_STAGE_ALL, bh);
     if (rc) return rc;
     rc = restart_stage(ctx, mp, ps, st);
     if (rc) return rc;
@@ -1952,7 +1982,7 @@
                       &ctx->smlvB, &ctx->smltmp, &ctx->flen, &ctx->fs, &ctx->rowsall, &ctx->rsbuf,
                       &ctx->rsplan, &ctx->rsbst, &ctx->pool_loc, &ctx->cbuf, &ctx->sids,
                       &ctx->logA, &ctx->logB, &ctx->logvA, &ctx->logvB, &ctx->tiebuf, &ctx->fk, &ctx->fkloc,
-                      &ctx->crbuf, &ctx->crcnt, &ctx->crlive, &ctx->crruns, &ctx->crall, &ctx->fsk, &ctx->bst2,
+                      &ctx->crbuf, &ctx->crcnt, &ctx->crlive, &ctx->crruns, &ctx->crall, &ctx->fsk,
                       &ctx->side, &ctx->bst8, &ctx->cbst, &ctx->dsarr, &ctx->labx, &ctx->rkpool0, &ctx->rkpool1,
                       &ctx->rku32, &ctx->ascii_all};
     for (DevBuf* b : bufs) b->release();
@@ -3820,6 +3850,13 @@
     HIPCHK(hipMemcpy(rec.data(), ctx->sorted_rec, N * 8, hipMemcpyDeviceToHost));
     HIPCHK(hipMemcpy(bkt.data(), ctx->sorted_buckets, P * 4, hipMemcpyDeviceToHost));
     HIPCHK(hipMemcpy(ids.data(), ctx->sorted_ids, P * 4, hipMemcpyDeviceToHost));
+    std::vector<bool> seen(P, false);
+    for (uint64_t i = 0; i < P; ++i) {
+        if (ids[i] >= P || seen[ids[i]] ||
+            (i && (bkt[i - 1] > bkt[i] || (bkt[i - 1] == bkt[i] && ids[i - 1] >= ids[i]))))
+            return fail(ctx, MUMS_E_HIP, "probe bucket partition out of order (internal error)");
+        seen[ids[i]] = true;
+    }
     std::vector<uint32_t> bucket_of_probe(P);
     for (uint64_t i = 0; i < P; ++i) bucket_of_probe[ids[i]] = bkt[i];
     for (uint64_t k = 0; k < P; ++k) {
diff --git a/libmems_amd/csrc/mums_internal.h b/libmems_amd/csrc/mums_internal.h
--- a/libmems_amd/csrc/mums_internal.h
+++ b/libmems_amd/csrc/mums_internal.h
@@ -197,7 +197,9 @@
                              const uint32_t* d_bstart, void* d_tmp, uint32_t* d_err, int* out_buf, hipStream_t st,
                              hipEvent_t* ev_ds = nullptr, int key_shift = 32, bool mask_parity = false,
                              bool key_runs = false, const uint32_t* hist_in = nullptr,
-                             const uint64_t* gsrc = nullptr, uint32_t* gout = nullptr);
+                             const uint64_t* gsrc = nullptr, uint32_t* gout = nullptr,
+                             const uint32_t* key32 = nullptr, uint32_t* out_keys = nullptr,
+                             uint32_t* out_ids = nullptr);
 size_t seg_parity_fix_tmp_bytes(uint64_t n);
 hipError_t seg_parity_fix(uint64_t* rec, uint64_t* scratch, uint64_t n, int key_bits, int msd_bits,
                           const uint32_t* d_bstart, void* d_tmp, uint32_t* d_err, hipStream_t st, int key_shift = 32);
@@ -217,9 +219,8 @@
                               uint32_t* slot_bucket, void* counters, hipStream_t st);
 hipError_t launch_probe_compact(uint64_t nblocks, const uint32_t* tile_count, const uint32_t* tile_off,
                                 const uint64_t* slot_info, const uint32_t* slot_bucket, uint64_t* probe_info,
-                                uint32_t* probe_bucket, hipStream_t st, bool packed);
-hipError_t launch_bucket_records(const uint32_t* b, uint64_t P, uint64_t* rec, hipStream_t st);
-hipError_t launch_bucket_split(const uint64_t* rec, uint64_t P, uint32_t* b, uint32_t* ids, hipStream_t st);
+                                uint32_t* probe_bucket, hipStream_t st, bool packed,
+                                uint32_t* bucket_hist = nullptr, int hist_passes = 0);
 template <int MG, typename View>
 hipError_t launch_materialize(View v, const uint64_t* probe_info, uint64_t P, const GenomeTable& gt,
                               const MatchParams& mp, int L, int64_t* rows, hipStream_t st, uint64_t* lkey = nullptr,
diff --git a/libmems_amd/csrc/radix_seg.hip b/libmems_amd/csrc/radix_seg.hip
--- a/libmems_amd/csrc/radix_seg.hip
+++ b/libmems_amd/csrc/radix_seg.hip
@@ -400,7 +400,8 @@
     }
 }
 
-template <int OB, int kIPT, bool kAlias = false, bool kLate = false, bool kGath = false, bool kHi = false>
+template <int OB, int kIPT, bool kAlias = false, bool kLate = false, bool kGath = false, bool kHi = false,
+          bool kKey32 = false, bool kSplit = false>
 __global__ __launch_bounds__(OB) __attribute__((amdgpu_waves_per_eu(OB == 768 ? 6 : 1)))
 void seg_onesweep_kernel(const uint64_t* __restrict__ rin,
                                                           uint64_t* __restrict__ rout,
@@ -412,9 +413,11 @@
                                                           const uint32_t* __restrict__ xq,
                                                           const uint64_t* __restrict__ gsrc = nullptr,
                                                           uint32_t* __restrict__ gout = nullptr,
-                                                          const uint4* __restrict__ xd = nullptr) {
+                                                          const uint4* __restrict__ xd = nullptr,
+                                                          uint32_t* __restrict__ gout2 = nullptr) {
     constexpr int kT = kIPT * OB;
     constexpr bool late = MUMS_OS_LATEPUB || kLate;
+    static_assert(!(kGath && kSplit), "one store form");
     constexpr int kW = OB / 64;
     static_assert(OB >= kDigits, "one thread per digit");
     static_assert(!kAlias || kW * kDigits * 4 <= kT * 8, "counts fit in the exchange buffer");
@@ -498,12 +501,18 @@
     const uint32_t pad = (uint32_t)kT - d.count;
     uint64_t key[kIPT];
     uint32_t rank[kIPT];
-    const char* tin = reinterpret_cast<const char*>(rin + d.start);
+    const char* tin = kKey32 ? reinterpret_cast<const char*>(reinterpret_cast<const uint32_t*>(rin) + d.start)
+                             : reinterpret_cast<const char*>(rin + d.start);
     auto loads = [&](auto full_c) {
         #pragma unroll
         for (int r = 0; r < kIPT; ++r) {
             const uint32_t q = qof(r);
             const bool in = decltype(full_c)::value || q < d.count;
+            if constexpr (kKey32) {
+                const uint32_t k32 = in ? *reinterpret_cast<const uint32_t*>(tin + q * 4u) : 0u;
+                key[r] = in ? ((uint64_t)k32 << 32) | ((uint32_t)d.start + q) : ~0ull;
+                continue;
+            }
 #if MUMS_SORT_NT & 1
             key[r] = in ? __builtin_nontemporal_load(reinterpret_cast<const uint64_t*>(tin + q * 8u)) : ~0ull;
 #else
@@ -634,7 +643,8 @@
     __syncthreads();
     OS_STAMP(5);
     uint64_t* bout = rout + bb;
-    uint32_t* bgout = kGath ? gout + bb : nullptr;
+    uint32_t* bgout = (kGath || kSplit) ? gout + bb : nullptr;
+    uint32_t* bgout2 = kSplit ? gout2 + bb : nullptr;
     auto stores = [&](auto full_c, auto far_c) {
         constexpr bool kFar = decltype(far_c)::value;
         #pragma unroll
@@ -652,6 +662,14 @@
                     const uint32_t gv = (uint32_t)gsrc[(uint32_t)k];
                     if constexpr (kFar) bgout[o] = gv;
                     else *reinterpret_cast<uint32_t*>(reinterpret_cast<char*>(bgout) + o * 4u) = gv;
+                } else if constexpr (kSplit) {
+                    if constexpr (kFar) {
+                        bgout[o] = (uint32_t)(k >> 32);
+                        bgout2[o] = (uint32_t)k;
+                    } else {
+                        *reinterpret_cast<uint32_t*>(reinterpret_cast<char*>(bgout) + o * 4u) = (uint32_t)(k >> 32);
+                        *reinterpret_cast<uint32_t*>(reinterpret_cast<char*>(bgout2) + o * 4u) = (uint32_t)k;
+                    }
                 } else {
                     uint64_t* op = kFar ? bout + o
                                         : reinterpret_cast<uint64_t*>(reinterpret_cast<char*>(bout) + o * 8u);
@@ -1275,15 +1293,21 @@
 hipError_t seg_onesweep_sort(uint64_t* recA, uint64_t* recB, uint64_t n, int key_bits, int msd_bits,
                              const uint32_t* d_bstart, void* d_tmp, uint32_t* d_err, int* out_buf, hipStream_t st,
                              hipEvent_t* ev_ds, int key_shift, bool mask_parity, bool key_runs,
-                             const uint32_t* hist_in, const uint64_t* gsrc, uint32_t* gout) {
+                             const uint32_t* hist_in, const uint64_t* gsrc, uint32_t* gout, const uint32_t* key32,
+                             uint32_t* out_keys, uint32_t* out_ids) {
     const int nkd = (key_bits + 7) / 8;
     const bool segfix = nkd >= 2 && seg_segfix_enabled();
     const int npass = segfix ? nkd - 1 : nkd;
     const int digit_shift = key_shift;
     if (segfix) key_shift += 8;
-    *out_buf = npass % 2;
+    const bool split = out_keys != nullptr;
+    *out_buf = split ? -1 : (npass + (key32 ? 1 : 0)) % 2;
     if (n == 0 || npass == 0) return hipSuccess;
     if (nkd > 4) return hipErrorInvalidValue;
+    if ((key32 || split) && (!key_runs || msd_bits != 0 || key_shift != 32 || gout || MUMS_SORT_PERSIST))
+        return hipErrorInvalidValue;
+    if (key32 && (!hist_in || segfix || MUMS_OS_NEXTHIST)) return hipErrorInvalidValue;
+    if (split && (segfix || !out_ids)) return hipErrorInvalidValue;
     const uint64_t nb = 1ull << msd_bits;
     const int tile = os_tile();
     const uint64_t ub = seg_tiles_upper(n, msd_bits, tile);
@@ -1344,8 +1368,8 @@
     (void)hipMemsetAsync(os_dev, 0, ub * 80, st);
     (void)hipMemcpyToSymbol(HIP_SYMBOL(g_os_stats), &os_dev, sizeof(os_dev), 0, hipMemcpyHostToDevice);
 #endif
-    uint64_t* src = recA;
-    uint64_t* dst = recB;
+    uint64_t* src = key32 ? reinterpret_cast<uint64_t*>(const_cast<uint32_t*>(key32)) : recA;
+    uint64_t* dst = key32 ? recA : recB;
     for (int p = 0; p < npass; ++p) {
         if (ev_ds) (void)hipEventRecord(ev_ds[2 * p], st);
 #if MUMS_SORT_PERSIST
@@ -1367,7 +1391,17 @@
         if (sh >= 32) MUMS_OS_LAUNCH1(OB, IPT, AL, true); \
         else MUMS_OS_LAUNCH1(OB, IPT, AL, false);       \
     } while (0)
-            if (key_runs && gout && p + 1 == npass) {
+            const bool k32 = key32 && p == 0, spl = split && p + 1 == npass;
+            if (k32 || spl) {
+#define MUMS_OS_LAUNCH_KI(K32, SPL)                                                                               \
+    hipLaunchKernelGGL((seg_onesweep_kernel<kSortBlock, kSortTile / kSortBlock, true, true, false, true, K32, SPL>), \
+                       dim3((unsigned)ub), dim3(kSortBlock), 0, st, src, dst, otiles, (uint32_t)ub, sh, p, npass,  \
+                       dbase, sp, tc, d_err, gn, xq, nullptr, out_keys, xd, out_ids)
+                if (k32 && spl) MUMS_OS_LAUNCH_KI(true, true);
+                else if (k32) MUMS_OS_LAUNCH_KI(true, false);
+                else MUMS_OS_LAUNCH_KI(false, true);
+#undef MUMS_OS_LAUNCH_KI
+            } else if (key_runs && gout && p + 1 == npass) {
                 hipLaunchKernelGGL((seg_onesweep_kernel<kSortBlock, kSortTile / kSortBlock, true, true, true>),
                                    dim3((unsigned)ub), dim3(kSortBlock), 0, st, src, dst, otiles, (uint32_t)ub, sh, p,
                                    npass, dbase, sp, tc, d_err, gn, xq, gsrc, gout, xd);
@@ -1429,7 +1463,7 @@
             hipLaunchKernelGGL(seg_dbase_kernel, dim3((unsigned)nb), dim3(kBlock), 0, st, ghist, d_bstart, npass,
                                dbase, p + 1);
         if (ev_ds) (void)hipEventRecord(ev_ds[2 * p + 1], st);
-        uint64_t* t = src;
+        uint64_t* t = (key32 && p == 0) ? recB : src;
         src = dst;
         dst = t;
     }
diff --git a/libmems_amd/csrc/replay.hip b/libmems_amd/csrc/replay.hip
--- a/libmems_amd/csrc/replay.hip
+++ b/libmems_amd/csrc/replay.hip
@@ -120,7 +120,7 @@
 }
 
 __global__ __launch_bounds__(kBlock) void chain_keys_kernel(const int64_t* __restrict__ pool, uint32_t nch, int G,
-                                                            uint32_t table_size, double inv_t,
+                                                            uint32_t table_size, uint64_t inv_t,
                                                             const uint32_t* __restrict__ bkey,
                                                             uint64_t* __restrict__ key_s, uint64_t* __restrict__ key_b) {
     const uint32_t c = blockIdx.x * kBlock + threadIdx.x;
@@ -1433,7 +1433,7 @@
     if (e != hipSuccess) return e;
     *bkey_out = bkey;
     hipLaunchKernelGGL(chain_keys_kernel, dim3(cgrid), dim3(kBlock), 0, st, pool, nch, gt.G, mp.table_size,
-                       1.0 / (double)mp.table_size, bkey, key_s, key_b);
+                       bucket_recip(mp.table_size), bkey, key_s, key_b);
     if ((e = hipGetLastError()) != hipSuccess) return e;
     int buf = 0;
     if ((e = radix_sort<uint64_t>(key_s, nullptr, nch, 32, kA, vA, kB, vB, d_radix_tmp, &buf, st)) != hipSuccess)
```
